# broadinstitute/permutect

Measured on AMD Instinct MI355X. Metric: read-sets/sec (train fwd+bwd), higher is better.
Workload: dtype f32 (fp32 accumulate; fwd: 2 x f16 pieces per operand = 23 bits; bwd: 2 x bf16 pieces = 16 bits)

## Files before the change

include/permutect_amd.h:

```cpp
#ifndef PERMUTECT_AMD_H
#define PERMUTECT_AMD_H

#include <stddef.h>
#include <stdint.h>

#ifdef __cplusplus
extern "C" {
#endif

#define PMT_ABI_VERSION 12

#define PMT_FAULT_JOIN 1
#define PMT_FAULT_F16_RANGE 2
#define PMT_FAULT_PLAN 4

#define PMT_OK 0
#define PMT_E_INVALID (-1)
#define PMT_E_UNSUPPORTED (-2)
#define PMT_E_CAPACITY (-3)
#define PMT_E_LAUNCH (-4)
#define PMT_E_WORKSPACE (-5)

#ifndef PMT_MAX_WIDTH
#define PMT_MAX_WIDTH 64
#endif
#ifndef PMT_MAX_HALF_FFN
#define PMT_MAX_HALF_FFN 16
#endif
#define PMT_MAX_CLUSTERS 16
#define PMT_MAX_OPS 8
#define PMT_MAX_ROW_INPUT 128
#define PMT_MAX_CNN_TAPS 192
#define PMT_ROWS_INFO 0
#define PMT_ROWS_ALT_COUNT 1
#define PMT_ROWS_SOURCE 2
#define PMT_MAX_SKIP_LAYERS 4
#define PMT_MAX_BLOCKS 16
#define PMT_MAX_LINEAR 96
#ifndef PMT_GROUP_WAVES
#define PMT_GROUP_WAVES 8
#endif
#define PMT_GROUP_TILES (2 * PMT_GROUP_WAVES)
#define PMT_GROUP_MAX_SETS (8 * PMT_GROUP_WAVES)
#define PMT_TILE 16

#define PMT_READS_PACKED_U8 0
#define PMT_READS_F16 1
#define PMT_READS_F32 2

typedef struct PmtLinear {
    int32_t in_dim, out_dim;
    int32_t w_frag;
    int32_t wt_frag;
    int32_t b_pvec;
    int32_t w_src;
    int32_t b_src;
    int32_t out_split;
    int32_t wb_frag;
    int32_t wtb_frag;
    int32_t wh_frag;
    int32_t emit_tab;
} PmtLinear;

#define PMT_OP_LINEAR 0
#define PMT_OP_SKIP 1
typedef struct PmtOp {
    int32_t kind;
    int32_t n_layers;
    int32_t selu_after;
    int32_t alpha_src;
    int32_t lin[PMT_MAX_SKIP_LAYERS];
} PmtOp;

typedef struct PmtMlp {
    int32_t n_ops, in_dim, out_dim;
    int32_t dropout;
    PmtOp ops[PMT_MAX_OPS];
} PmtMlp;

typedef struct PmtBlock {
    int32_t norm_w_pvec, norm_b_pvec;
    int32_t norm_w_src, norm_b_src;
    int32_t proj1[2], proj2[2];
    int32_t sgu_norm_w_pvec, sgu_norm_b_pvec;
    int32_t sgu_norm_w_src, sgu_norm_b_src;
    int32_t alpha_src[2], beta_src[2];
    int32_t gamma_src;
    int32_t ref_reg_pvec, ref_reg_src;
    int32_t reg_weight_phi;
} PmtBlock;

typedef struct PmtHead {
    int32_t stdev_e_phi;
    int32_t dirs_ke_phi;
    int32_t art_stdev_k_phi;
    int32_t log_w_k_phi;
    int32_t mu_k_src;
    int32_t sigma_k_phi;
    int32_t lambda_k_phi;
    int32_t reserved;
} PmtHead;

#define PMT_MAX_CNN_LAYERS 12
#define PMT_CNN_CONV 0
#define PMT_CNN_POOL 1
#define PMT_CNN_LEAKY_RELU 2
#define PMT_CNN_SELU 3
#define PMT_CNN_FLATTEN 4
#define PMT_CNN_LINEAR 5
typedef struct PmtCnnLayer {
    int32_t kind;
    int32_t in_ch, in_len, out_ch, out_len;
    int32_t kernel, stride, padding, dilation;
    int32_t w_src, b_src;
    int32_t in_off, out_off;
    int32_t lin;
    int32_t reserved[2];
} PmtCnnLayer;
typedef struct PmtCnn {
    int32_t n_layers;
    int32_t seq_len;
    int32_t out_dim;
    int32_t max_act;
    int32_t sum_act;
    int32_t reserved[3];
    PmtCnnLayer layers[PMT_MAX_CNN_LAYERS];
} PmtCnn;

typedef struct PmtModel {
    int32_t abi_version;
    int32_t num_read_features;
    int32_t read_embed_dim;
    int32_t variant_embed_dim;
    int32_t d_model;
    int32_t d_ffn;
    int32_t num_blocks;
    int32_t feature_dim;
    int32_t num_clusters;
    int32_t n_linear;
    int32_t theta_size, phi_size, packed_size;
    int32_t translation_src;
    int32_t translation_pvec;
    int32_t rotation_lin;
    PmtMlp read_mlp;
    PmtMlp reducer;
    PmtMlp row_mlp[3];
    PmtBlock blocks[PMT_MAX_BLOCKS];
    PmtHead head;
    PmtCnn cnn;
    PmtLinear lin[PMT_MAX_LINEAR];
    int32_t force_shape;
    int32_t force_cnn;
    int32_t cnn_debug;
    int32_t emit_base;
    int32_t emit_len;
    float dropout_p;
} PmtModel;

typedef struct PmtBatch {
    int32_t num_variants;
    int32_t num_groups;
    int32_t read_format;
    int32_t read_row_bytes;
    const void* reads;
    const int64_t* read_index;
    const int32_t* ref_offsets;
    const int32_t* alt_offsets;
    const float* variant_embed;
    const int32_t* group_start;
    const int32_t* group_tile_base;
    int64_t total_tiles;
    int32_t* debug_flags;
    const int32_t* group_span;
    const int32_t* num_groups_dev;
    const int32_t* set_groups;
    uint64_t dropout_seed;
    int32_t* join_fault;
} PmtBatch;

typedef struct PmtOutputs {
    float* logits_b;
    float* logits_bk;
    float* features_be;
    float* ref_features_be;
} PmtOutputs;

typedef struct PmtOutputGrads {
    const float* d_logits_b;
    const float* d_logits_bk;
    const float* d_features_be;
    const float* d_ref_features_be;
} PmtOutputGrads;

typedef struct PmtAdamW {
    float lr, beta1, beta2, eps, weight_decay, max_grad_norm;
    int32_t step;
    int32_t reserved;
} PmtAdamW;
#define PMT_STEP_ON_DEVICE (-1)
#define PMT_STEP_SLOT 1000


int pmt_abi_version(void);

int pmt_shape_info(int32_t* nine);
int pmt_shape_id(const struct PmtModel* m);
int pmt_limits(int32_t* four);

int pmt_build_id(char* out, int32_t capacity);

int pmt_struct_bytes(int which);

int pmt_model_check(const PmtModel* model);

#define PMT_PHI_EXP 0
#define PMT_PHI_BOUNDED 1
#define PMT_PHI_UNIT_ROWS 2
#define PMT_PHI_LOG_SOFTMAX 3
#define PMT_PHI_ORTHOGONAL 4
#define PMT_MAX_PHI_SEGS 48
#define PMT_MAX_ORTHO_DIM 32
typedef struct PmtPhiSeg {
    int32_t kind, theta_off, phi_off, rows, cols, reserved;
    float p0, p1;
    int32_t base_rs, base_cs;
    const float* base;
} PmtPhiSeg;
typedef struct PmtPhiProgram {
    int32_t n_segs, reserved;
    PmtPhiSeg seg[PMT_MAX_PHI_SEGS];
} PmtPhiProgram;

int pmt_phi_forward(const PmtPhiProgram* prog, const float* theta, float* phi, void* stream);
int pmt_phi_backward(const PmtPhiProgram* prog, const float* theta, const float* phi, const float* grad_phi,
                     float* grad_theta, void* stream);

typedef struct PmtIntColumn {
    const void* ptr;
    int64_t stride;
    int32_t elem_bytes, reserved;
} PmtIntColumn;

typedef struct PmtBinning {
    int32_t num_sources, num_variant_types, num_ref_bins, num_alt_bins, count_bin_skip, max_ref_count, max_alt_count, reserved;
} PmtBinning;

typedef struct PmtDownsample {
    int32_t num_variants;
    int32_t reference_alt_gather;
    uint64_t seed;
    int64_t force_random;
    const int32_t* ref_offsets;
    const int32_t* alt_offsets;
    const float* ref_weights_b4;
    const float* alt_weights_b4;
    const float* ref_fracs_in;
    const float* alt_fracs_in;
    const float* ref_weight_table;
    const float* alt_weight_table;
    PmtIntColumn labels, variant_types, sources;
    PmtBinning bins;
} PmtDownsample;
int pmt_downsample_counts(const PmtDownsample* args, float* ref_fracs, float* alt_fracs, int32_t* new_ref_counts,
                          int32_t* new_alt_counts, void* stream);
int pmt_downsample_index(const PmtDownsample* args, const float* ref_fracs, const float* alt_fracs,
                         const int32_t* new_ref_offsets, const int32_t* new_alt_offsets, int64_t* read_index, void* stream);

#define PMT_FIT_MAX_STEPS 200000
int pmt_downsample_fit(const float* counts_slvra, int32_t num_sources, const float* ref_trans_kry, const float* alt_trans_haz,
                       float* ref_logits_slvrak, float* alt_logits_slvrah, int32_t steps, double lr, double beta1, double beta2,
                       double eps, double weight_decay, float* loss_before_after, void* stream);

int pmt_spectra_fit(const int32_t* variant_types, const int32_t* depths, const int32_t* alt_counts, int32_t n, float* log_alpha_dv,
                    float* log_beta_dv, int32_t batch_size, int32_t epochs, double lr, double beta1, double beta2, double eps,
                    void* stream);

#define PMT_POSTERIOR_RAW 80
#define PMT_POSTERIOR_PARTIAL 128
typedef struct PmtPosteriorRows {
    int64_t n;
    const int32_t *variant_types, *depths, *alt_counts, *normal_depths, *normal_alt_counts, *contexts;
    const float *seq_error_log_lks, *normal_seq_error_log_lks, *allele_frequencies, *mafs, *normal_mafs, *artifact_logits;
} PmtPosteriorRows;
typedef struct PmtPosteriorParams {
    const float *log_priors_vc, *snv_log_priors_rrra, *raw;
    int32_t use_context, no_germline, has_het_beta;
    float het_beta;
} PmtPosteriorParams;
int pmt_posterior_forward(const PmtPosteriorRows* rows, int64_t first, int64_t count, const PmtPosteriorParams* params, float* log_priors_bc,
                          float* spectra_log_lks_bc, float* normal_log_lks_bc, float* log_posteriors_bc, void* stream);
int pmt_posterior_step(const PmtPosteriorRows* rows, int64_t first, int64_t count, const PmtPosteriorParams* params, float* partials,
                       int32_t num_partial_rows, void* stream);
int pmt_posterior_update(const float* partials, int32_t num_partial_rows, int64_t count, float* raw, float* adam_m, float* adam_v, int64_t step,
                         double lr, double beta1, double beta2, double eps, float* totals_tc, double* loss_sum, void* stream);

typedef struct PmtLossArgs {
    int32_t num_variants, num_clusters, num_sources, reserved;
    float max_outlier_logit;
    float max_alt_count;
    const float* logits_b;
    const float* logits_bk;
    const float* alt_count_raw;
    const float* source_logits;
    const int64_t* labels;
    int64_t label_stride;
    const int64_t* alt_counts;
    int64_t alt_count_stride;
    const int64_t* sources;
    int64_t source_stride;
    const float* weights;
    const float* source_weights;
} PmtLossArgs;
typedef struct PmtLossOutputs {
    float* supervised_b;
    float* unsupervised_b;
    float* alt_count_b;
    float* source_b;
    float* total_b;
} PmtLossOutputs;
typedef struct PmtLossInputGrads {
    float* d_logits_b;
    float* d_logits_bk;
    float* d_alt_count_raw;
    float* d_source_logits;
} PmtLossInputGrads;
int pmt_losses_forward(const PmtLossArgs* args, const PmtLossOutputs* out, void* stream);
int pmt_losses_backward(const PmtLossArgs* args, const PmtLossOutputs* grad_out, const PmtLossInputGrads* grad_in, void* stream);

typedef struct PmtRecordArgs {
    int32_t num_variants, num_bins;
    int32_t num_variant_types, num_ref_bins, num_alt_bins, count_bin_skip, max_ref_count, max_alt_count;
    PmtIntColumn labels, variant_types, sources, ref_counts, alt_counts;
    const float* weights;
    const float* source_weights;
    const float* supervised_b;
    const float* unsupervised_b;
    const float* alt_count_b;
    const float* source_b;
} PmtRecordArgs;
int pmt_record_losses(const PmtRecordArgs* args, float* histograms, void* stream);

typedef struct PmtEvalArgs {
    int32_t num_variants, epoch_index;
    int32_t num_logit_bins, min_logit, max_logit, logit_bin_skip;
    PmtBinning bins;
    PmtIntColumn labels, variant_types, sources, ref_counts, alt_counts;
    const float* logits_b;
    const float* weights_b;
    int64_t nhist;
} PmtEvalArgs;
int pmt_record_evaluation(const PmtEvalArgs* args, float* flat, void* stream);

typedef struct PmtBalanceArgs {
    int32_t num_variants, recompute;
    float attenuation;
    int32_t reserved;
    PmtBinning bins;
    PmtIntColumn labels, variant_types, sources, ref_counts, alt_counts;
    const float* logits_b;
    float* counts;
    float* pseudo_counts;
    const float* weights_in;
    const float* unlabeled_weights_in;
    const float* source_weights_in;
    float* weights_out;
    float* unlabeled_weights_out;
    float* source_weights_out;
    float* weights_b;
    float* source_weights_b;
} PmtBalanceArgs;
int pmt_balance_step(const PmtBalanceArgs* args, void* stream);

int pmt_posterior_rows(const float* float_rows, int64_t float_stride, int32_t n_scalars, int32_t logit_col, const float* logits_b,
                       const float* features_be, int32_t e, const int64_t* dest_ids, int32_t n, float* block, int64_t block_stride,
                       void* stream);

int pmt_plan_groups(const int32_t* ref_counts, const int32_t* alt_counts, int32_t num_variants,
                    int32_t* group_start, int32_t* group_tile_base, int32_t* bad_variant);

int pmt_plan_groups_device(const int32_t* ref_offsets, const int32_t* alt_offsets, int32_t num_variants, int32_t* group_start,
                           int32_t* group_tile_base, int32_t capacity, int32_t* num_groups_dev, int32_t* fault, int32_t* scratch,
                           void* stream);
int pmt_plan_device_chunks(int32_t num_variants);

int pmt_pack_order(const int32_t* ref_counts, const int32_t* alt_counts, int32_t num_variants, int32_t window, int32_t* order);
int pmt_pack_order_batches(const int32_t* ref_counts, const int32_t* alt_counts, int32_t num_variants, int32_t batch,
                           int32_t window, int32_t threads, int32_t* order);

int pmt_plan_groups_split(const int32_t* ref_counts, const int32_t* alt_counts, int32_t num_variants, int32_t* span,
                          int32_t* tile_base, int32_t max_groups, int32_t* needs_layered);

size_t pmt_layered_scratch_floats(const PmtModel* model, int64_t total_tiles, int32_t num_variants);

int pmt_forward_layered(const PmtModel* model_host, const PmtModel* model_dev, const float* theta, const float* phi,
                        const float* packed, const PmtBatch* batch, const PmtOutputs* out, float* stash, float* scratch,
                        void* stream);

size_t pmt_layered_backward_scratch_floats(const PmtModel* model, int64_t total_tiles, int32_t num_variants);

int pmt_backward_layered(const PmtModel* model_host, const PmtModel* model_dev, const float* theta, const float* phi,
                         const float* packed, const PmtBatch* batch, const PmtOutputs* out, const PmtOutputGrads* dout,
                         const float* stash, float* scratch, float* grad_theta, float* grad_phi, float* grad_variant_embed,
                         float* grad_partials, int32_t num_partials, void* stream);

size_t pmt_stash_bytes(const PmtModel* model, int64_t total_tiles, int32_t num_variants);


int pmt_pack_params(const PmtModel* model_host, const PmtModel* model_dev, const float* theta, const float* phi,
                    float* packed, void* stream);

int pmt_scan_counts(const void* ref_counts, const void* alt_counts, int32_t count_elem_bytes, int64_t count_stride,
                    int32_t num_variants, int32_t* ref_offsets, int32_t* alt_offsets, void* stream);

int pmt_build_read_index(const int64_t* row_start, const int32_t* ref_offsets, const int32_t* alt_offsets,
                         int32_t num_variants, int64_t* read_index, void* stream);

int pmt_compose_batch(const int16_t* chunk_ints, int32_t int_cols, const void* chunk_floats_f16, int32_t float_cols,
                      const int64_t* chunk_row_start, const int64_t* ids, int32_t num_variants, int32_t ref_col, int32_t alt_col,
                      int64_t* int_tensor, float* float_tensor, int64_t* row_start, int32_t* ref_offsets, int32_t* alt_offsets,
                      int64_t* read_index, void* stream);
int pmt_compose_batch_planned(const int16_t* chunk_ints, int32_t int_cols, const void* chunk_floats_f16, int32_t float_cols,
                              const int64_t* chunk_row_start, const int64_t* ids, int32_t num_variants,
                              const int32_t* ref_offsets, const int32_t* alt_offsets, int64_t* int_tensor, float* float_tensor,
                              int64_t* row_start, int64_t* read_index, void* stream);

int pmt_host_copy(void* dst, const void* src, size_t bytes, int32_t threads);
int pmt_host_copy_rows(void* dst, const void* src, int64_t rows, int64_t row_bytes, int64_t zero_offset, int64_t zero_bytes,
                       int32_t threads);
int pmt_prepare_chunk(const int16_t* ints, int64_t row_stride, int32_t ref_col, int32_t alt_col, int32_t n, int32_t shuffle,
                      uint64_t seed, int32_t batch, int32_t window, int32_t threads, int32_t* ref_host, int32_t* alt_host,
                      int64_t* ids, int32_t* plans, int64_t plans_capacity, int32_t* batch_info, int32_t* offsets);

int pmt_forward(const PmtModel* model_host, const PmtModel* model_dev, const float* theta, const float* phi,
                const float* packed, const PmtBatch* batch, const PmtOutputs* out, float* stash, void* stream);

int pmt_backward(const PmtModel* model_host, const PmtModel* model_dev, const float* theta, const float* phi,
                 const float* packed, const PmtBatch* batch, const PmtOutputs* out, const PmtOutputGrads* dout,
                 const float* stash, float* grad_theta, float* grad_phi, float* grad_variant_embed, float* grad_partials,
                 int32_t num_partials, void* stream);

int pmt_dropout_mask(uint64_t seed, float p, int32_t lin, int64_t row0, int64_t rows, int32_t width, float* out);

size_t pmt_rows_stash_bytes(const PmtModel* model, int which, int32_t n_rows);
int pmt_rows_forward(const PmtModel* model_host, const PmtModel* model_dev, int which, const float* theta,
                     const float* packed, const float* in, int64_t in_stride, int32_t n_rows, float* out,
                     int64_t out_stride, float* stash, uint64_t dropout_seed, void* stream);
int pmt_rows_backward(const PmtModel* model_host, const PmtModel* model_dev, int which, const float* theta,
                      const float* packed, const float* in, int64_t in_stride, int32_t n_rows, const float* d_out,
                      int64_t d_out_stride, const float* stash, float* grad_theta, float* d_in, int64_t d_in_stride,
                      float d_in_scale, float* workspace, size_t workspace_floats, uint64_t dropout_seed, void* stream);
size_t pmt_rows_workspace_floats(const PmtModel* model_host, int which);

int pmt_cnn_forward(const PmtModel* model_host, const PmtModel* model_dev, const float* theta, const float* packed,
                    const int64_t* haplotypes, int64_t hap_stride, int32_t n, float* out, int64_t out_stride, float* stash,
                    void* stream);
size_t pmt_cnn_stash_floats(const PmtModel* model_host);
int pmt_cnn_backward(const PmtModel* model_host, const PmtModel* model_dev, const float* theta, const float* packed,
                     const int64_t* haplotypes, int64_t hap_stride, int32_t n, const float* d_out, int64_t d_out_stride,
                     const float* stash, float* grad_theta, float* workspace, size_t workspace_floats, void* stream);
size_t pmt_cnn_workspace_floats(const PmtModel* model_host);

int pmt_clip_adamw(float* theta, const float* grad, float* exp_avg, float* exp_avg_sq, int64_t n,
                   const PmtAdamW* hyper, float* scratch, float* grad_norm_out, void* stream);

#ifdef __cplusplus
}
#endif
#endif
```

permutect_amd/architecture/artifact_model.py:

```python
from __future__ import annotations

from typing import Optional

import torch
from torch import Tensor, nn

from permutect_amd import constants
from permutect_amd.architecture import modules as M
from permutect_amd.data.batch import Batch
from permutect_amd.data.datum import Data
from permutect_amd.engine import lib as L
from permutect_amd.engine.runtime import (HaplotypeCnnFunction, LossesFunction, PhiFunction, ReadSetEngine, ReadSetFunction,
                                          RowsMlpFunction, VariantEmbedFunction)
from permutect_amd.enums import Epoch
from permutect_amd.parameters import ModelParameters, install_pickle_alias

_BCE = nn.BCEWithLogitsLoss(reduction="none")


def gpu_if_available() -> torch.device:
    return torch.device("cuda" if torch.cuda.is_available() else "cpu")


class BatchOutput:

    def __init__(self, features_be: Tensor, ref_features_be: Tensor, logits_b: Tensor, logits_bk: Tensor,
                 weights: Tensor, source_weights: Tensor):
        self.features_be = features_be
        self.ref_features_be = ref_features_be
        self.logits_b = logits_b
        self.logits_bk = logits_bk
        self.weights = weights
        self.source_weights = source_weights

    @property
    def artifact_probs_b(self) -> Tensor:
        return torch.sigmoid(self.logits_b)

    @property
    def outlier_binary_logits(self) -> Tensor:
        lk = self.logits_bk
        nonoutlier = torch.logsumexp(torch.cat((lk[:, 0:1], lk[:, 2:]), dim=-1), dim=-1)
        return lk[:, 1] - nonoutlier


class BatchLosses:

    def __init__(self, supervised_losses_b, unsupervised_losses_b, alt_count_losses_b, source_prediction_losses_b,
                 total_losses_b):
        self.supervised_losses_b = supervised_losses_b
        self.unsupervised_losses_b = unsupervised_losses_b
        self.alt_count_losses_b = alt_count_losses_b
        self.source_prediction_losses_b = source_prediction_losses_b
        self.total_losses_b = total_losses_b
        self.total_loss = torch.sum(total_losses_b)


class SetMeansView:

    def __init__(self, means_be: Tensor, lengths_b: Tensor):
        self._means, self.lengths_b = means_be, lengths_b

    def means_over_sets(self) -> Tensor:
        return self._means

    def batch_size(self) -> int:
        return len(self.lengths_b)


class ArtifactModel(nn.Module):
    def __init__(self, params: ModelParameters, num_read_features: int, num_info_features: int,
                 haplotypes_length: int, device=None):
        super().__init__()
        if device is None:
            device = gpu_if_available()
        self._device = torch.device(device)
        if self._device.type == "cuda" and self._device.index is None:
            self._device = torch.device("cuda", torch.cuda.current_device())
        self._dtype = torch.float32
        self._haplotypes_length = haplotypes_length
        self._params = params

        self.read_embedding = M.MLP([num_read_features] + params.read_layers, params.batch_normalize, params.dropout_p)
        self.info_embedding = M.MLP([num_info_features] + params.info_layers, params.batch_normalize, params.dropout_p)
        self.haplotypes_cnn = M.DNASequenceConvolution(params.ref_seq_layer_strings, haplotypes_length // 2)
        embedding_dim = (self.read_embedding.output_dimension() + self.info_embedding.output_dimension()
                         + self.haplotypes_cnn.output_dimension())
        self.ref_alt_reads_encoder = M.GatedRefAltMLP(embedding_dim, params.self_attention_hidden_dimension,
                                                      params.num_self_attention_layers)
        self.reducer = M.MLP([embedding_dim] + params.aggregation_layers, params.batch_normalize, params.dropout_p)
        e = self.reducer.output_dimension()
        self.pre_clustering_transform = M.EuclideanTransformation(e)
        self.feature_clustering = M.FeatureClustering(e, params.num_artifact_clusters)
        self.alt_count_predictor = M.Adversarial(M.MLP([e] + [30, -1, -1, -1, 1]), adversarial_strength=0.01)
        self.alt_count_loss_func = nn.MSELoss(reduction="none")
        self.source_predictor = M.Adversarial(M.MLP([e] + [1], params.batch_normalize, params.dropout_p), 0.01)
        self.num_sources = 1

        self.to(device=self._device, dtype=self._dtype)
        self._engine: Optional[ReadSetEngine] = None

    def engine(self) -> ReadSetEngine:
        if self._engine is None:
            with torch.inference_mode(False):
                self._engine = ReadSetEngine(self, self._device)
        return self._engine

    def _invalidate_engine(self):
        self._engine = None

    def reset_source_predictor(self, num_sources: int = 1):
        hidden = [] if num_sources == 1 else [-1, -1]
        layers = [self.reducer.output_dimension()] + hidden + [num_sources]
        self.source_predictor = M.Adversarial(
            M.MLP(layers, self._params.batch_normalize, self._params.dropout_p), 0.01
        ).to(device=self._device, dtype=self._dtype)
        self.num_sources = num_sources
        self._invalidate_engine()

    def ref_alt_seq_embedding_dimension(self) -> int:
        return self.haplotypes_cnn.output_dimension()

    def haplotypes_length(self) -> int:
        return self._haplotypes_length

    def calibration_parameters(self):
        fc = self.feature_clustering
        return [fc.parametrizations.nonartifact_stdev_e.original, fc.parametrizations.artifact_stdev_k.original]

    def set_epoch_type(self, epoch_type: Epoch):
        train = epoch_type == Epoch.TRAIN
        self.train(train)
        for p in self.parameters():
            p.requires_grad_(train)

    def forward(self, batch: Batch):
        pass

    def variant_embedding(self, batch: Batch) -> Tensor:
        eng = self.engine()
        return VariantEmbedFunction.apply(eng, batch.get_info_be(), batch.get_haplotypes_bs(), eng.trigger)

    def _cnn_has_batchnorm(self) -> bool:
        flag = self.__dict__.get("_cnn_bn_flag")
        if flag is None:
            flag = self.__dict__["_cnn_bn_flag"] = any(isinstance(m, nn.BatchNorm1d) for m in self.haplotypes_cnn.modules())
        return flag

    def _encode(self, batch: Batch):
        if self.training and self._cnn_has_batchnorm():
            raise NotImplementedError("permutect_amd runs a haplotype CNN with batch_norm tokens in eval mode only (model.eval() under "
                                      "no_grad / inference_mode: filter_variants, evaluation); training with BatchNorm statistics is not built")
        if self.training and self._params.batch_normalize:
            raise NotImplementedError("permutect_amd runs a batch_normalize model in eval mode only (model.eval(): filter_variants, "
                                      "evaluation); training with BatchNorm statistics is not built")
        eng = self.engine()
        eng.draw_dropout_seed(self.training)
        if batch.size() == 0:
            d, dev = eng.plan.desc, self._device
            z = lambda *shape: torch.zeros(*shape, dtype=torch.float32, device=dev)
            return (z(0), z(0, d.num_clusters + 2), z(0, d.feature_dim), z(0, d.feature_dim)), z(0, d.variant_embed_dim)
        key = None if torch.is_grad_enabled() else eng.params_key()
        if key is not None and eng.packed_for is not None and eng.packed_for[0] == key:
            phi = eng.packed_for[1]
        else:
            prog = eng.plan.phi_program(self)
            phi = eng.plan.materialize_phi(self) if prog is None else PhiFunction.apply(eng, prog, eng.trigger)
            eng.pack(phi.detach().contiguous())
            eng.packed_for = (key, phi.detach()) if (key is not None and not torch.is_grad_enabled()) else None
        variant_embed = self.variant_embedding(batch)
        outs = ReadSetFunction.apply(eng, batch, phi, variant_embed)
        return outs, variant_embed

    def calculate_features(self, batch: Batch, weight_range: float = 0):
        (logits_b, logits_bk, feats, ref_feats), ve = self._encode(batch)
        e_hap = self.haplotypes_cnn.output_dimension()
        return (SetMeansView(ref_feats, batch.get(Data.REF_COUNT)), SetMeansView(feats, batch.get(Data.ALT_COUNT)),
                ve[:, ve.shape[1] - e_hap:])

    def compute_batch_output(self, batch: Batch, balancer=None) -> BatchOutput:
        (logits_b, logits_bk, feats, ref_feats), _ = self._encode(batch)
        if balancer is None:
            weights_b = source_weights = torch.ones_like(logits_b)
        elif logits_b.is_cuda and hasattr(balancer, "weights_from_logits"):
            weights_b, source_weights = balancer.weights_from_logits(batch, logits_b)
        else:
            weights_b, source_weights_b = balancer.process_batch_and_compute_weights(
                batch, artifact_probs_b=torch.sigmoid(logits_b).detach())
            source_weights = weights_b * source_weights_b
        return BatchOutput(features_be=feats, ref_features_be=ref_feats, logits_b=logits_b, logits_bk=logits_bk,
                           weights=weights_b, source_weights=source_weights)

    def compute_source_prediction_losses(self, features_be: Tensor, batch: Batch) -> Tensor:
        if self.num_sources > 1:
            eng = self.engine()
            logits = RowsMlpFunction.apply(eng, L.ROWS_SOURCE, features_be, eng.trigger,
                                           float(self.source_predictor.gradient_reversal.alpha))
            probs = torch.softmax(logits, dim=-1)
            targets = torch.nn.functional.one_hot(batch.get(Data.SOURCE).long(), self.num_sources)
            return torch.sum(torch.square(probs - targets), dim=-1)
        return torch.zeros(batch.size(), device=self._device, dtype=self._dtype)

    def compute_alt_count_losses(self, features_be: Tensor, batch: Batch) -> Tensor:
        eng = self.engine()
        raw = RowsMlpFunction.apply(eng, L.ROWS_ALT_COUNT, features_be, eng.trigger,
                                    float(self.alt_count_predictor.gradient_reversal.alpha))
        pred = torch.sigmoid(raw.view(-1))
        target = batch.get(Data.ALT_COUNT).to(dtype=pred.dtype) / constants.MAX_ALT_COUNT
        return self.alt_count_loss_func(pred, target)

    def compute_batch_losses(self, output: BatchOutput, batch: Batch) -> BatchLosses:
        eng = self.engine()
        alt_raw = RowsMlpFunction.apply(eng, L.ROWS_ALT_COUNT, output.features_be, eng.trigger,
                                        float(self.alt_count_predictor.gradient_reversal.alpha))
        source_logits, sources = None, None
        if self.num_sources > 1:
            source_logits = RowsMlpFunction.apply(eng, L.ROWS_SOURCE, output.features_be, eng.trigger,
                                                  float(self.source_predictor.gradient_reversal.alpha))
            sources = batch.get(Data.SOURCE).long()
        sup, unsup, alt, src, total = LossesFunction.apply(
            eng, output.logits_b, output.logits_bk, alt_raw, source_logits, batch.get(Data.LABEL).long(),
            batch.get(Data.ALT_COUNT).long(), sources, output.weights, output.source_weights)
        return BatchLosses(sup, unsup, alt, src, total)

    def compute_batch_losses_torch(self, output: BatchOutput, batch: Batch) -> BatchLosses:
        labels_b = batch.get_training_labels()
        is_labeled_b = batch.get_is_labeled_mask()
        supervised = is_labeled_b * _BCE(output.logits_b, labels_b)
        clipped = torch.clip(output.outlier_binary_logits, max=constants.MAX_OUTLIER_LOGIT)
        unsupervised = (1 - is_labeled_b) * _BCE(clipped, torch.zeros_like(clipped))
        alt_count = self.compute_alt_count_losses(output.features_be, batch)
        source = self.compute_source_prediction_losses(output.features_be, batch)
        total = output.weights * (supervised + unsupervised + alt_count) + output.source_weights * source
        return BatchLosses(supervised, unsupervised, alt_count, source, total)

    def make_dict_for_saving(self, artifact_log_priors=None, artifact_spectra=None):
        state = {k: v.detach().clone() for k, v in self.state_dict().items()}
        return {
            constants.STATE_DICT_NAME: state,
            constants.HYPERPARAMS_NAME: self._params,
            constants.NUM_READ_FEATURES_NAME: self.read_embedding.input_dimension(),
            constants.NUM_INFO_FEATURES_NAME: self.info_embedding.input_dimension(),
            constants.REF_SEQUENCE_LENGTH_NAME: self.haplotypes_length(),
            constants.ARTIFACT_LOG_PRIORS_NAME: artifact_log_priors,
            constants.ARTIFACT_SPECTRA_STATE_DICT_NAME: None if artifact_spectra is None else artifact_spectra.state_dict(),
        }

    def save_model(self, path, artifact_log_priors=None, artifact_spectra=None):
        self.reset_source_predictor()
        install_pickle_alias()
        torch.save(self.make_dict_for_saving(artifact_log_priors, artifact_spectra), path)


def load_model(path, device: torch.device = None):
    if device is None:
        device = gpu_if_available()
    install_pickle_alias()
    with torch.serialization.safe_globals([ModelParameters]):
        saved = torch.load(path, map_location=device, weights_only=True)
    model = ArtifactModel(saved[constants.HYPERPARAMS_NAME], num_read_features=saved[constants.NUM_READ_FEATURES_NAME],
                          num_info_features=saved[constants.NUM_INFO_FEATURES_NAME],
                          haplotypes_length=saved[constants.REF_SEQUENCE_LENGTH_NAME], device=device)
    model.load_state_dict(saved[constants.STATE_DICT_NAME])
    model.to(model._dtype)
    return model, saved[constants.ARTIFACT_LOG_PRIORS_NAME], saved[constants.ARTIFACT_SPECTRA_STATE_DICT_NAME]
```

permutect_amd/csrc/pmt_losses.hip:

```cpp
#include <hip/hip_runtime.h>
#include <math.h>

#include "permutect_amd.h"

#define LOSS_THREADS 256

__device__ __forceinline__ float softplus_f(float x) { return fmaxf(x, 0.f) + log1pf(expf(-fabsf(x))); }
__device__ __forceinline__ float sigmoid_f(float x) { return 1.0f / (1.0f + expf(-x)); }

struct OutlierLogit {
    float o;
    float mx, se;
};
__device__ __forceinline__ OutlierLogit outlier_logit(const float* __restrict__ lk, int K) {
    OutlierLogit r;
    r.mx = lk[0];
    for (int k = 0; k < K; ++k) r.mx = fmaxf(r.mx, lk[2 + k]);
    r.se = expf(lk[0] - r.mx);
    for (int k = 0; k < K; ++k) r.se += expf(lk[2 + k] - r.mx);
    r.o = lk[1] - (r.mx + logf(r.se));
    return r;
}

__global__ __launch_bounds__(LOSS_THREADS) void pmt_losses_forward_kernel(PmtLossArgs a, PmtLossOutputs out) {
    const int b = blockIdx.x * LOSS_THREADS + threadIdx.x;
    if (b >= a.num_variants) return;
    const int K = a.num_clusters, S = a.num_sources;
    const long long label = a.labels[(size_t)b * a.label_stride];
    const float is_labeled = label != 2 ? 1.f : 0.f;
    const float target = label == 0 ? 1.f : (label == 2 ? 0.5f : 0.f);
    const float x = a.logits_b[b];
    const float sup = is_labeled * (fmaxf(x, 0.f) - x * target + log1pf(expf(-fabsf(x))));
    const OutlierLogit ol = outlier_logit(a.logits_bk + (size_t)b * (K + 2), K);
    const float unsup = (1.f - is_labeled) * softplus_f(fminf(ol.o, a.max_outlier_logit));
    const float pred = sigmoid_f(a.alt_count_raw[b]);
    const float tgt = (float)a.alt_counts[(size_t)b * a.alt_count_stride] / a.max_alt_count;
    const float altl = (pred - tgt) * (pred - tgt);
    float src = 0.f;
    if (S > 1 && a.source_logits != nullptr) {
        const float* sl = a.source_logits + (size_t)b * S;
        const long long sid = a.sources[(size_t)b * a.source_stride];
        float mx = sl[0];
        for (int s = 1; s < S; ++s) mx = fmaxf(mx, sl[s]);
        float se = 0.f;
        for (int s = 0; s < S; ++s) se += expf(sl[s] - mx);
        for (int s = 0; s < S; ++s) {
            const float d = expf(sl[s] - mx) / se - (s == sid ? 1.f : 0.f);
            src += d * d;
        }
    }
    out.supervised_b[b] = sup;
    out.unsupervised_b[b] = unsup;
    out.alt_count_b[b] = altl;
    out.source_b[b] = src;
    out.total_b[b] = a.weights[b] * (sup + unsup + altl) + a.source_weights[b] * src;
}

__global__ __launch_bounds__(LOSS_THREADS) void pmt_losses_backward_kernel(PmtLossArgs a, PmtLossOutputs g, PmtLossInputGrads d) {
    const int b = blockIdx.x * LOSS_THREADS + threadIdx.x;
    if (b >= a.num_variants) return;
    const int K = a.num_clusters, S = a.num_sources;
    const float gt = g.total_b ? g.total_b[b] : 0.f;
    const float g_sup = (g.supervised_b ? g.supervised_b[b] : 0.f) + gt * a.weights[b];
    const float g_unsup = (g.unsupervised_b ? g.unsupervised_b[b] : 0.f) + gt * a.weights[b];
    const float g_alt = (g.alt_count_b ? g.alt_count_b[b] : 0.f) + gt * a.weights[b];
    const float g_src = (g.source_b ? g.source_b[b] : 0.f) + gt * a.source_weights[b];
    const long long label = a.labels[(size_t)b * a.label_stride];
    const float is_labeled = label != 2 ? 1.f : 0.f;
    const float target = label == 0 ? 1.f : (label == 2 ? 0.5f : 0.f);
    d.d_logits_b[b] = g_sup * is_labeled * (sigmoid_f(a.logits_b[b]) - target);
    const float* lk = a.logits_bk + (size_t)b * (K + 2);
    float* dlk = d.d_logits_bk + (size_t)b * (K + 2);
    const OutlierLogit ol = outlier_logit(lk, K);
    const float go = ol.o <= a.max_outlier_logit ? g_unsup * (1.f - is_labeled) * sigmoid_f(ol.o) : 0.f;
    dlk[1] = go;
    dlk[0] = -go * expf(lk[0] - ol.mx) / ol.se;
    for (int k = 0; k < K; ++k) dlk[2 + k] = -go * expf(lk[2 + k] - ol.mx) / ol.se;
    const float pred = sigmoid_f(a.alt_count_raw[b]);
    const float tgt = (float)a.alt_counts[(size_t)b * a.alt_count_stride] / a.max_alt_count;
    d.d_alt_count_raw[b] = g_alt * 2.f * (pred - tgt) * pred * (1.f - pred);
    if (S > 1 && a.source_logits != nullptr && d.d_source_logits != nullptr) {
        const float* sl = a.source_logits + (size_t)b * S;
        float* dsl = d.d_source_logits + (size_t)b * S;
        const long long sid = a.sources[(size_t)b * a.source_stride];
        float mx = sl[0];
        for (int s = 1; s < S; ++s) mx = fmaxf(mx, sl[s]);
        float se = 0.f;
        for (int s = 0; s < S; ++s) se += expf(sl[s] - mx);
        float dot = 0.f;
        for (int s = 0; s < S; ++s) {
            const float p = expf(sl[s] - mx) / se;
            dot += 2.f * (p - (s == sid ? 1.f : 0.f)) * p;
        }
        for (int s = 0; s < S; ++s) {
            const float p = expf(sl[s] - mx) / se;
            dsl[s] = g_src * (2.f * (p - (s == sid ? 1.f : 0.f)) * p - p * dot);
        }
    }
}

static int loss_args_check(const PmtLossArgs* a) {
    if (!a || a->num_variants < 0 || a->num_clusters < 0 || a->num_clusters > PMT_MAX_CLUSTERS || a->num_sources < 1) return PMT_E_INVALID;
    if (a->num_variants == 0) return PMT_OK;
    if (!a->logits_b || !a->logits_bk || !a->alt_count_raw || !a->labels || !a->alt_counts || !a->weights || !a->source_weights)
        return PMT_E_INVALID;
    if (a->num_sources > 1 && a->source_logits && !a->sources) return PMT_E_INVALID;
    return PMT_OK;
}

extern "C" int pmt_losses_forward(const PmtLossArgs* args, const PmtLossOutputs* out, void* stream) {
    const int rc = loss_args_check(args);
    if (rc) return rc;
    if (!out || !out->supervised_b || !out->unsupervised_b || !out->alt_count_b || !out->source_b || !out->total_b) return PMT_E_INVALID;
    if (args->num_variants == 0) return PMT_OK;
    hipLaunchKernelGGL(pmt_losses_forward_kernel, dim3((args->num_variants + LOSS_THREADS - 1) / LOSS_THREADS), dim3(LOSS_THREADS), 0,
                       reinterpret_cast<hipStream_t>(stream), *args, *out);
    return hipGetLastError() == hipSuccess ? PMT_OK : PMT_E_LAUNCH;
}

extern "C" int pmt_losses_backward(const PmtLossArgs* args, const PmtLossOutputs* grad_out, const PmtLossInputGrads* grad_in,
                                   void* stream) {
    const int rc = loss_args_check(args);
    if (rc) return rc;
    if (!grad_out || !grad_in || !grad_in->d_logits_b || !grad_in->d_logits_bk || !grad_in->d_alt_count_raw) return PMT_E_INVALID;
    if (args->num_variants == 0) return PMT_OK;
    hipLaunchKernelGGL(pmt_losses_backward_kernel, dim3((args->num_variants + LOSS_THREADS - 1) / LOSS_THREADS), dim3(LOSS_THREADS), 0,
                       reinterpret_cast<hipStream_t>(stream), *args, *grad_out, *grad_in);
    return hipGetLastError() == hipSuccess ? PMT_OK : PMT_E_LAUNCH;
}

#define REC_THREADS 256
#define REC_MAX_BINS 2048

__device__ __forceinline__ long long rec_col_at(const PmtIntColumn& c, int i) {
    if (c.ptr == nullptr) return 0;
    return c.elem_bytes == 8 ? reinterpret_cast<const long long*>(c.ptr)[(size_t)i * c.stride]
                             : (long long)reinterpret_cast<const int*>(c.ptr)[(size_t)i * c.stride];
}

__global__ __launch_bounds__(REC_THREADS) void pmt_record_losses_kernel(PmtRecordArgs a, float* __restrict__ hist) {
    __shared__ float sh[6][REC_MAX_BINS];
    const int nb = a.num_bins;
    for (int i = threadIdx.x; i < 6 * REC_MAX_BINS; i += REC_THREADS) (&sh[0][0])[i] = 0.f;
    __syncthreads();
    const int b = blockIdx.x * REC_THREADS + threadIdx.x;
    if (b < a.num_variants) {
        const long long label = rec_col_at(a.labels, b), vt = rec_col_at(a.variant_types, b), src = rec_col_at(a.sources, b);
        const long long nr = rec_col_at(a.ref_counts, b), na = rec_col_at(a.alt_counts, b);
        const int rbin = (int)min(nr, (long long)a.max_ref_count) / a.count_bin_skip;
        const int abin = ((int)min(na, (long long)a.max_alt_count) - 1) / a.count_bin_skip;
        const int idx = (int)((((src * 3 + label) * a.num_variant_types + vt) * a.num_ref_bins + rbin) * a.num_alt_bins + abin);
        if (idx >= 0 && idx < nb) {
            const float is_labeled = label != 2 ? 1.f : 0.f;
            const float w = a.weights[b], sw = a.source_weights[b];
            const float lw = is_labeled * w, uw = (1.f - is_labeled) * w;
            atomicAdd(&sh[0][idx], a.supervised_b[b] * lw + a.unsupervised_b[b] * uw);
            atomicAdd(&sh[1][idx], lw + uw);
            atomicAdd(&sh[2][idx], a.alt_count_b[b] * w);
            atomicAdd(&sh[3][idx], w);
            atomicAdd(&sh[4][idx], a.source_b[b] * sw);
            atomicAdd(&sh[5][idx], sw);
        }
    }
    __syncthreads();
    for (int i = threadIdx.x; i < 6 * nb; i += REC_THREADS) {
        const int hsel = i / nb, j = i - hsel * nb;
        const float v = sh[hsel][j];
        if (v != 0.f) atomicAdd(&hist[(size_t)hsel * nb + j], v);
    }
}

extern "C" int pmt_record_losses(const PmtRecordArgs* args, float* histograms, void* stream) {
    if (!args || !histograms || args->num_variants < 0 || args->num_bins < 1 || args->num_bins > REC_MAX_BINS) return PMT_E_INVALID;
    if (args->num_variants == 0) return PMT_OK;
    for (const PmtIntColumn* c : {&args->labels, &args->variant_types, &args->sources, &args->ref_counts, &args->alt_counts})
        if (c->ptr != nullptr && c->elem_bytes != 4 && c->elem_bytes != 8) return PMT_E_INVALID;
    if (!args->labels.ptr || !args->variant_types.ptr || !args->ref_counts.ptr || !args->alt_counts.ptr || !args->weights || !args->source_weights ||
        !args->supervised_b || !args->unsupervised_b || !args->alt_count_b || !args->source_b || args->count_bin_skip < 1)
        return PMT_E_INVALID;
    hipLaunchKernelGGL(pmt_record_losses_kernel, dim3((args->num_variants + REC_THREADS - 1) / REC_THREADS), dim3(REC_THREADS), 0,
                       reinterpret_cast<hipStream_t>(stream), *args, histograms);
    return hipGetLastError() == hipSuccess ? PMT_OK : PMT_E_LAUNCH;
}

__global__ __launch_bounds__(256) void pmt_posterior_rows_kernel(const float* __restrict__ float_rows, long long float_stride, int n_scalars,
                                                                 int logit_col, const float* __restrict__ logits_b,
                                                                 const float* __restrict__ features_be, int e,
                                                                 const long long* __restrict__ dest_ids, int n, float* __restrict__ block,
                                                                 long long block_stride) {
    const int width = n_scalars + e;
    for (long long i = (long long)blockIdx.x * 256 + threadIdx.x; i < (long long)n * width; i += (long long)gridDim.x * 256) {
        const int v = (int)(i / width), c = (int)(i - (long long)v * width);
        const long long row = dest_ids ? dest_ids[v] : v;
        float x;
        if (c < n_scalars) {
            const float raw = c == logit_col ? logits_b[v] : float_rows[(long long)v * float_stride + c];
            x = (float)(_Float16)raw;
        } else {
            x = features_be[(long long)v * e + (c - n_scalars)];
        }
        block[row * block_stride + c] = x;
    }
}

extern "C" int pmt_posterior_rows(const float* float_rows, int64_t float_stride, int32_t n_scalars, int32_t logit_col, const float* logits_b,
                                  const float* features_be, int32_t e, const int64_t* dest_ids, int32_t n, float* block, int64_t block_stride,
                                  void* stream) {
    if (!float_rows || !logits_b || !features_be || !block || n < 0 || n_scalars < 1 || e < 0 || logit_col < 0 || logit_col >= n_scalars ||
        block_stride < n_scalars + e)
        return PMT_E_INVALID;
    if (n == 0) return PMT_OK;
    const long long work = (long long)n * (n_scalars + e);
    const int grid = (int)((work + 255) / 256 < 4096 ? (work + 255) / 256 : 4096);
    hipLaunchKernelGGL(pmt_posterior_rows_kernel, dim3(grid), dim3(256), 0, reinterpret_cast<hipStream_t>(stream), float_rows, (long long)float_stride,
                       n_scalars, logit_col, logits_b, features_be, e, reinterpret_cast<const long long*>(dest_ids), n, block, (long long)block_stride);
    return hipGetLastError() == hipSuccess ? PMT_OK : PMT_E_LAUNCH;
}
```

permutect_amd/csrc/pmt_phi.hip:

```cpp
#include <hip/hip_runtime.h>
#include <math.h>

#include "permutect_amd.h"

#define PHI_THREADS 256
#define PHI_MAXN (2 * PMT_MAX_ORTHO_DIM)

__device__ double block_max(double v, double* red) {
    const int tid = threadIdx.x;
    red[tid] = v;
    __syncthreads();
    for (int s = PHI_THREADS / 2; s > 0; s >>= 1) {
        if (tid < s) red[tid] = fmax(red[tid], red[tid + s]);
        __syncthreads();
    }
    const double r = red[0];
    __syncthreads();
    return r;
}
__device__ double block_sum(double v, double* red) {
    const int tid = threadIdx.x;
    red[tid] = v;
    __syncthreads();
    for (int s = PHI_THREADS / 2; s > 0; s >>= 1) {
        if (tid < s) red[tid] += red[tid + s];
        __syncthreads();
    }
    const double r = red[0];
    __syncthreads();
    return r;
}

__device__ void matmul(double* __restrict__ Cm, const double* __restrict__ A, const double* __restrict__ B, int N, double scale) {
    for (int idx = threadIdx.x; idx < N * N; idx += PHI_THREADS) {
        const int i = idx / N, j = idx - i * N;
        double a0 = 0.0, a1 = 0.0, a2 = 0.0, a3 = 0.0;
        const double* ar = A + i * N;
        const double* bc = B + j;
        int k = 0;
        for (; k + 3 < N; k += 4) {
            a0 += ar[k] * bc[k * N];
            a1 += ar[k + 1] * bc[(k + 1) * N];
            a2 += ar[k + 2] * bc[(k + 2) * N];
            a3 += ar[k + 3] * bc[(k + 3) * N];
        }
        for (; k < N; ++k) a0 += ar[k] * bc[k * N];
        Cm[idx] = ((a0 + a1) + (a2 + a3)) * scale;
    }
    __syncthreads();
}

__device__ void expm_inplace(double* S, double* B, double* P, double* T, int N, double* red) {
    double colsum = 0.0;
    if (threadIdx.x < N)
        for (int i = 0; i < N; ++i) colsum += fabs(S[i * N + threadIdx.x]);
    const double norm1 = block_max(colsum, red);
    int s = 0;
    if (norm1 > 0.5) s = (int)ceil(log2(norm1 / 0.5));
    const double scale = ldexp(1.0, -s);
    for (int idx = threadIdx.x; idx < N * N; idx += PHI_THREADS) {
        const double b = S[idx] * scale;
        B[idx] = b;
        P[idx] = b;
        const int i = idx / N, j = idx - i * N;
        S[idx] = b + (i == j ? 1.0 : 0.0);
    }
    __syncthreads();
    for (int k = 2; k <= 12; ++k) {
        matmul(T, P, B, N, 1.0 / (double)k);
        for (int idx = threadIdx.x; idx < N * N; idx += PHI_THREADS) {
            P[idx] = T[idx];
            S[idx] += T[idx];
        }
        __syncthreads();
    }
    for (int q = 0; q < s; ++q) {
        matmul(T, S, S, N, 1.0);
        for (int idx = threadIdx.x; idx < N * N; idx += PHI_THREADS) S[idx] = T[idx];
        __syncthreads();
    }
}

struct PhiShared {
    double m[4][PHI_MAXN * PHI_MAXN];
    double red[PHI_THREADS];
};
static_assert(sizeof(PhiShared) <= 160 * 1024, "LDS budget");

__global__ __launch_bounds__(PHI_THREADS) void pmt_phi_forward_kernel(PmtPhiProgram prog, const float* __restrict__ theta,
                                                                       float* __restrict__ phi) {
    __shared__ __attribute__((aligned(16))) PhiShared sh;
    const PmtPhiSeg sg = prog.seg[blockIdx.x];
    const float* x = theta + sg.theta_off;
    float* y = phi + sg.phi_off;
    const int tid = threadIdx.x, n = sg.rows * sg.cols;
    if (sg.kind == PMT_PHI_EXP) {
        for (int i = tid; i < n; i += PHI_THREADS) y[i] = expf(x[i]);
    } else if (sg.kind == PMT_PHI_BOUNDED) {
        for (int i = tid; i < n; i += PHI_THREADS) y[i] = sg.p1 * (1.0f / (1.0f + expf(-x[i]))) + sg.p0;
    } else if (sg.kind == PMT_PHI_UNIT_ROWS) {
        for (int r = 0; r < sg.rows; ++r) {
            double q = 0.0;
            for (int i = tid; i < sg.cols; i += PHI_THREADS) q += (double)x[r * sg.cols + i] * (double)x[r * sg.cols + i];
            const float norm = (float)sqrt(block_sum(q, sh.red));
            for (int i = tid; i < sg.cols; i += PHI_THREADS) y[r * sg.cols + i] = x[r * sg.cols + i] / norm;
        }
    } else if (sg.kind == PMT_PHI_LOG_SOFTMAX) {
        for (int r = 0; r < sg.rows; ++r) {
            double mx = -INFINITY;
            for (int i = tid; i < sg.cols; i += PHI_THREADS) mx = fmax(mx, (double)x[r * sg.cols + i]);
            mx = block_max(mx, sh.red);
            double se = 0.0;
            for (int i = tid; i < sg.cols; i += PHI_THREADS) se += exp((double)x[r * sg.cols + i] - mx);
            const double lse = mx + log(block_sum(se, sh.red));
            for (int i = tid; i < sg.cols; i += PHI_THREADS) y[r * sg.cols + i] = (float)((double)x[r * sg.cols + i] - lse);
        }
    } else if (sg.kind == PMT_PHI_ORTHOGONAL) {
        const int N = sg.rows;
        double* S = sh.m[0];
        for (int idx = tid; idx < N * N; idx += PHI_THREADS) {
            const int i = idx / N, j = idx - i * N;
            S[idx] = i > j ? (double)x[i * N + j] : (i < j ? -(double)x[j * N + i] : 0.0);
        }
        __syncthreads();
        expm_inplace(S, sh.m[1], sh.m[2], sh.m[3], N, sh.red);
        for (int idx = tid; idx < N * N; idx += PHI_THREADS) {
            const int i = idx / N, j = idx - i * N;
            double acc = 0.0;
            if (sg.base != nullptr) {
                for (int k = 0; k < N; ++k) acc += (double)sg.base[i * sg.base_rs + k * sg.base_cs] * S[k * N + j];
            } else {
                acc = S[idx];
            }
            y[idx] = (float)acc;
        }
    }
}

__global__ __launch_bounds__(PHI_THREADS) void pmt_phi_backward_kernel(PmtPhiProgram prog, const float* __restrict__ theta,
                                                                        const float* __restrict__ phi,
                                                                        const float* __restrict__ gphi,
                                                                        float* __restrict__ gtheta) {
    __shared__ __attribute__((aligned(16))) PhiShared sh;
    const PmtPhiSeg sg = prog.seg[blockIdx.x];
    const float* x = theta + sg.theta_off;
    const float* y = phi + sg.phi_off;
    const float* gy = gphi + sg.phi_off;
    float* gx = gtheta + sg.theta_off;
    const int tid = threadIdx.x, n = sg.rows * sg.cols;
    if (sg.kind == PMT_PHI_EXP) {
        for (int i = tid; i < n; i += PHI_THREADS) gx[i] += gy[i] * y[i];
    } else if (sg.kind == PMT_PHI_BOUNDED) {
        for (int i = tid; i < n; i += PHI_THREADS) {
            const float s = 1.0f / (1.0f + expf(-x[i]));
            gx[i] += gy[i] * sg.p1 * s * (1.0f - s);
        }
    } else if (sg.kind == PMT_PHI_UNIT_ROWS) {
        for (int r = 0; r < sg.rows; ++r) {
            double q = 0.0, d = 0.0;
            for (int i = tid; i < sg.cols; i += PHI_THREADS) {
                q += (double)x[r * sg.cols + i] * (double)x[r * sg.cols + i];
                d += (double)y[r * sg.cols + i] * (double)gy[r * sg.cols + i];
            }
            const double norm = sqrt(block_sum(q, sh.red));
            const double dot = block_sum(d, sh.red);
            for (int i = tid; i < sg.cols; i += PHI_THREADS)
                gx[r * sg.cols + i] += (float)(((double)gy[r * sg.cols + i] - (double)y[r * sg.cols + i] * dot) / norm);
        }
    } else if (sg.kind == PMT_PHI_LOG_SOFTMAX) {
        for (int r = 0; r < sg.rows; ++r) {
            double g = 0.0;
            for (int i = tid; i < sg.cols; i += PHI_THREADS) g += (double)gy[r * sg.cols + i];
            const double gsum = block_sum(g, sh.red);
            for (int i = tid; i < sg.cols; i += PHI_THREADS)
                gx[r * sg.cols + i] += (float)((double)gy[r * sg.cols + i] - exp((double)y[r * sg.cols + i]) * gsum);
        }
    } else if (sg.kind == PMT_PHI_ORTHOGONAL) {
        const int nn = sg.rows, N = 2 * nn;
        double* S = sh.m[0];
        double* G = sh.m[1];
        for (int idx = tid; idx < nn * nn; idx += PHI_THREADS) {
            const int i = idx / nn, j = idx - i * nn;
            double acc = 0.0;
            if (sg.base != nullptr) {
                for (int k = 0; k < nn; ++k) acc += (double)sg.base[k * sg.base_rs + i * sg.base_cs] * (double)gy[k * nn + j];
            } else {
                acc = (double)gy[idx];
            }
            G[idx] = acc;
        }
        __syncthreads();
        for (int idx = tid; idx < N * N; idx += PHI_THREADS) {
            const int i = idx / N, j = idx - i * N;
            const int bi = i % nn, bj = j % nn;
            double v = 0.0;
            if ((i < nn) == (j < nn)) {
                v = bi > bj ? -(double)x[bi * nn + bj] : (bi < bj ? (double)x[bj * nn + bi] : 0.0);
            } else if (i < nn) {
                v = G[bi * nn + bj];
            }
            S[idx] = v;
        }
        __syncthreads();
        double* B = sh.m[1];
        expm_inplace(S, B, sh.m[2], sh.m[3], N, sh.red);
        for (int idx = tid; idx < nn * nn; idx += PHI_THREADS) {
            const int i = idx / nn, j = idx - i * nn;
            if (i > j) gx[idx] += (float)(S[i * N + nn + j] - S[j * N + nn + i]);
        }
    }
}

static int phi_check(const PmtPhiProgram* p) {
    if (!p || p->n_segs < 0 || p->n_segs > PMT_MAX_PHI_SEGS) return PMT_E_INVALID;
    for (int i = 0; i < p->n_segs; ++i) {
        const PmtPhiSeg* s = &p->seg[i];
        if (s->kind < PMT_PHI_EXP || s->kind > PMT_PHI_ORTHOGONAL || s->rows < 1 || s->cols < 1 || s->theta_off < 0 || s->phi_off < 0)
            return PMT_E_INVALID;
        if (s->kind == PMT_PHI_ORTHOGONAL && (s->rows != s->cols || s->rows > PMT_MAX_ORTHO_DIM)) return PMT_E_UNSUPPORTED;
    }
    return PMT_OK;
}

extern "C" int pmt_phi_forward(const PmtPhiProgram* prog, const float* theta, float* phi, void* stream) {
    const int rc = phi_check(prog);
    if (rc) return rc;
    if (!theta || !phi) return PMT_E_INVALID;
    if (prog->n_segs == 0) return PMT_OK;
    hipLaunchKernelGGL(pmt_phi_forward_kernel, dim3(prog->n_segs), dim3(PHI_THREADS), 0, reinterpret_cast<hipStream_t>(stream),
                       *prog, theta, phi);
    return hipGetLastError() == hipSuccess ? PMT_OK : PMT_E_LAUNCH;
}

extern "C" int pmt_phi_backward(const PmtPhiProgram* prog, const float* theta, const float* phi, const float* grad_phi,
                                float* grad_theta, void* stream) {
    const int rc = phi_check(prog);
    if (rc) return rc;
    if (!theta || !phi || !grad_phi || !grad_theta) return PMT_E_INVALID;
    if (prog->n_segs == 0) return PMT_OK;
    hipLaunchKernelGGL(pmt_phi_backward_kernel, dim3(prog->n_segs), dim3(PHI_THREADS), 0, reinterpret_cast<hipStream_t>(stream),
                       *prog, theta, phi, grad_phi, grad_theta);
    return hipGetLastError() == hipSuccess ? PMT_OK : PMT_E_LAUNCH;
}
```

permutect_amd/engine/lib.py:

```python
from __future__ import annotations

import ctypes as C
import os

_HERE = os.path.dirname(os.path.dirname(os.path.abspath(__file__)))
LIB_PATH = os.environ.get("PMT_LIB", os.path.join(_HERE, "libpermutect_amd.so"))

ABI_VERSION = 12
MAX_WIDTH, MAX_HALF_FFN, MAX_CLUSTERS = 64, 16, 16
MAX_HALF_FFN_WIDE = 32
MAX_WIDTH_WIDE = 128
MAX_ROW_INPUT = 128
MAX_CNN_TAPS = 192
ROWS_INFO, ROWS_ALT_COUNT, ROWS_SOURCE = 0, 1, 2
MAX_OPS, MAX_SKIP_LAYERS, MAX_BLOCKS, MAX_LINEAR = 8, 4, 16, 96
GROUP_WAVES = int(os.environ.get("PMT_GROUP_WAVES", 8))
GROUP_TILES, GROUP_MAX_SETS, TILE = 2 * GROUP_WAVES, 8 * GROUP_WAVES, 16
READS_PACKED_U8, READS_F16, READS_F32 = 0, 1, 2
OP_LINEAR, OP_SKIP = 0, 1
SLOT_FLOATS = 4 * 256

POSTERIOR_RAW, POSTERIOR_PARTIAL = 80, 128

STEP_ON_DEVICE, STEP_SLOT = -1, 1000
E_INVALID, E_UNSUPPORTED, E_CAPACITY, E_LAUNCH, E_WORKSPACE = -1, -2, -3, -4, -5
_ERR = {-1: "invalid argument/descriptor", -2: "configuration not supported by the gfx950 kernels",
        -3: "a read set exceeds the register-resident group capacity", -4: "HIP launch failure",
        -5: "workspace too small"}

i32, i64, vp = C.c_int32, C.c_int64, C.c_void_p


class PmtLinear(C.Structure):
    _fields_ = [("in_dim", i32), ("out_dim", i32), ("w_frag", i32), ("wt_frag", i32), ("b_pvec", i32),
                ("w_src", i32), ("b_src", i32), ("out_split", i32), ("wb_frag", i32), ("wtb_frag", i32), ("wh_frag", i32), ("emit_tab", i32)]


class PmtOp(C.Structure):
    _fields_ = [("kind", i32), ("n_layers", i32), ("selu_after", i32), ("alpha_src", i32),
                ("lin", i32 * MAX_SKIP_LAYERS)]


class PmtMlp(C.Structure):
    _fields_ = [("n_ops", i32), ("in_dim", i32), ("out_dim", i32), ("dropout", i32), ("ops", PmtOp * MAX_OPS)]


class PmtBlock(C.Structure):
    _fields_ = [("norm_w_pvec", i32), ("norm_b_pvec", i32), ("norm_w_src", i32), ("norm_b_src", i32),
                ("proj1", i32 * 2), ("proj2", i32 * 2),
                ("sgu_norm_w_pvec", i32), ("sgu_norm_b_pvec", i32), ("sgu_norm_w_src", i32), ("sgu_norm_b_src", i32),
                ("alpha_src", i32 * 2), ("beta_src", i32 * 2), ("gamma_src", i32),
                ("ref_reg_pvec", i32), ("ref_reg_src", i32), ("reg_weight_phi", i32)]


class PmtHead(C.Structure):
    _fields_ = [("stdev_e_phi", i32), ("dirs_ke_phi", i32), ("art_stdev_k_phi", i32), ("log_w_k_phi", i32),
                ("mu_k_src", i32), ("sigma_k_phi", i32), ("lambda_k_phi", i32), ("reserved", i32)]


MAX_CNN_LAYERS = 12
CNN_CONV, CNN_POOL, CNN_LEAKY_RELU, CNN_SELU, CNN_FLATTEN, CNN_LINEAR = range(6)


class PmtCnnLayer(C.Structure):
    _fields_ = [("kind", i32), ("in_ch", i32), ("in_len", i32), ("out_ch", i32), ("out_len", i32),
                ("kernel", i32), ("stride", i32), ("padding", i32), ("dilation", i32), ("w_src", i32), ("b_src", i32),
                ("in_off", i32), ("out_off", i32), ("lin", i32), ("reserved", i32 * 2)]


class PmtCnn(C.Structure):
    _fields_ = [("n_layers", i32), ("seq_len", i32), ("out_dim", i32), ("max_act", i32), ("sum_act", i32),
                ("reserved", i32 * 3), ("layers", PmtCnnLayer * MAX_CNN_LAYERS)]


class PmtModel(C.Structure):
    _fields_ = [("abi_version", i32), ("num_read_features", i32), ("read_embed_dim", i32),
                ("variant_embed_dim", i32), ("d_model", i32), ("d_ffn", i32), ("num_blocks", i32),
                ("feature_dim", i32), ("num_clusters", i32), ("n_linear", i32),
                ("theta_size", i32), ("phi_size", i32), ("packed_size", i32),
                ("translation_src", i32), ("translation_pvec", i32), ("rotation_lin", i32),
                ("read_mlp", PmtMlp), ("reducer", PmtMlp), ("row_mlp", PmtMlp * 3), ("blocks", PmtBlock * MAX_BLOCKS), ("head", PmtHead), ("cnn", PmtCnn),
                ("lin", PmtLinear * MAX_LINEAR),
                ("force_shape", i32), ("force_cnn", i32), ("cnn_debug", i32), ("emit_base", i32), ("emit_len", i32),
                ("dropout_p", C.c_float)]


class PmtBatch(C.Structure):
    _fields_ = [("num_variants", i32), ("num_groups", i32), ("read_format", i32), ("read_row_bytes", i32),
                ("reads", vp), ("read_index", vp), ("ref_offsets", vp), ("alt_offsets", vp), ("variant_embed", vp),
                ("group_start", vp), ("group_tile_base", vp), ("total_tiles", i64), ("debug_flags", vp), ("group_span", vp),
                ("num_groups_dev", vp), ("set_groups", vp), ("dropout_seed", C.c_uint64), ("join_fault", vp)]


class PmtOutputs(C.Structure):
    _fields_ = [("logits_b", vp), ("logits_bk", vp), ("features_be", vp), ("ref_features_be", vp)]


class PmtOutputGrads(C.Structure):
    _fields_ = [("d_logits_b", vp), ("d_logits_bk", vp), ("d_features_be", vp), ("d_ref_features_be", vp)]


class PmtAdamW(C.Structure):
    _fields_ = [("lr", C.c_float), ("beta1", C.c_float), ("beta2", C.c_float), ("eps", C.c_float),
                ("weight_decay", C.c_float), ("max_grad_norm", C.c_float), ("step", i32), ("reserved", i32)]


PHI_EXP, PHI_BOUNDED, PHI_UNIT_ROWS, PHI_LOG_SOFTMAX, PHI_ORTHOGONAL = range(5)
MAX_PHI_SEGS, MAX_ORTHO_DIM = 48, 32


class PmtPhiSeg(C.Structure):
    _fields_ = [("kind", i32), ("theta_off", i32), ("phi_off", i32), ("rows", i32), ("cols", i32), ("reserved", i32),
                ("p0", C.c_float), ("p1", C.c_float), ("base_rs", i32), ("base_cs", i32), ("base", vp)]


class PmtPhiProgram(C.Structure):
    _fields_ = [("n_segs", i32), ("reserved", i32), ("seg", PmtPhiSeg * MAX_PHI_SEGS)]


class PmtIntColumn(C.Structure):
    _fields_ = [("ptr", vp), ("stride", i64), ("elem_bytes", i32), ("reserved", i32)]


class PmtBinning(C.Structure):
    _fields_ = [("num_sources", i32), ("num_variant_types", i32), ("num_ref_bins", i32), ("num_alt_bins", i32),
                ("count_bin_skip", i32), ("max_ref_count", i32), ("max_alt_count", i32), ("reserved", i32)]


def int_column(t) -> PmtIntColumn:
    c = PmtIntColumn()
    if t is None:
        return c
    assert t.dim() == 1 and t.element_size() in (4, 8) and not t.is_floating_point(), (t.shape, t.dtype)
    c.ptr, c.stride, c.elem_bytes = t.data_ptr(), (t.stride(0) if t.numel() > 1 else 1), t.element_size()
    return c


class PmtDownsample(C.Structure):
    _fields_ = [("num_variants", i32), ("reference_alt_gather", i32), ("seed", C.c_uint64), ("force_random", i64),
                ("ref_offsets", vp), ("alt_offsets", vp), ("ref_weights_b4", vp), ("alt_weights_b4", vp),
                ("ref_fracs_in", vp), ("alt_fracs_in", vp), ("ref_weight_table", vp), ("alt_weight_table", vp),
                ("labels", PmtIntColumn), ("variant_types", PmtIntColumn), ("sources", PmtIntColumn), ("bins", PmtBinning)]


class PmtBalanceArgs(C.Structure):
    _fields_ = [("num_variants", i32), ("recompute", i32), ("attenuation", C.c_float), ("reserved", i32), ("bins", PmtBinning),
                ("labels", PmtIntColumn), ("variant_types", PmtIntColumn), ("sources", PmtIntColumn), ("ref_counts", PmtIntColumn),
                ("alt_counts", PmtIntColumn), ("logits_b", vp), ("counts", vp), ("pseudo_counts", vp),
                ("weights_in", vp), ("unlabeled_weights_in", vp), ("source_weights_in", vp),
                ("weights_out", vp), ("unlabeled_weights_out", vp), ("source_weights_out", vp),
                ("weights_b", vp), ("source_weights_b", vp)]


class PmtEvalArgs(C.Structure):
    _fields_ = [("num_variants", i32), ("epoch_index", i32), ("num_logit_bins", i32), ("min_logit", i32), ("max_logit", i32),
                ("logit_bin_skip", i32), ("bins", PmtBinning), ("labels", PmtIntColumn), ("variant_types", PmtIntColumn),
                ("sources", PmtIntColumn), ("ref_counts", PmtIntColumn), ("alt_counts", PmtIntColumn), ("logits_b", vp), ("weights_b", vp),
                ("nhist", i64)]


class PmtRecordArgs(C.Structure):
    _fields_ = [("num_variants", i32), ("num_bins", i32), ("num_variant_types", i32), ("num_ref_bins", i32),
                ("num_alt_bins", i32), ("count_bin_skip", i32), ("max_ref_count", i32), ("max_alt_count", i32),
                ("labels", PmtIntColumn), ("variant_types", PmtIntColumn), ("sources", PmtIntColumn), ("ref_counts", PmtIntColumn),
                ("alt_counts", PmtIntColumn), ("weights", vp), ("source_weights", vp),
                ("supervised_b", vp), ("unsupervised_b", vp), ("alt_count_b", vp), ("source_b", vp)]


class PmtLossArgs(C.Structure):
    _fields_ = [("num_variants", i32), ("num_clusters", i32), ("num_sources", i32), ("reserved", i32),
                ("max_outlier_logit", C.c_float), ("max_alt_count", C.c_float),
                ("logits_b", vp), ("logits_bk", vp), ("alt_count_raw", vp), ("source_logits", vp),
                ("labels", vp), ("label_stride", i64), ("alt_counts", vp), ("alt_count_stride", i64),
                ("sources", vp), ("source_stride", i64), ("weights", vp), ("source_weights", vp)]


class PmtLossOutputs(C.Structure):
    _fields_ = [("supervised_b", vp), ("unsupervised_b", vp), ("alt_count_b", vp), ("source_b", vp), ("total_b", vp)]


class PmtLossInputGrads(C.Structure):
    _fields_ = [("d_logits_b", vp), ("d_logits_bk", vp), ("d_alt_count_raw", vp), ("d_source_logits", vp)]


class PmtPosteriorRows(C.Structure):
    _fields_ = [("n", i64), ("variant_types", vp), ("depths", vp), ("alt_counts", vp), ("normal_depths", vp), ("normal_alt_counts", vp),
                ("contexts", vp), ("seq_error_log_lks", vp), ("normal_seq_error_log_lks", vp), ("allele_frequencies", vp), ("mafs", vp),
                ("normal_mafs", vp), ("artifact_logits", vp)]


class PmtPosteriorParams(C.Structure):
    _fields_ = [("log_priors_vc", vp), ("snv_log_priors_rrra", vp), ("raw", vp), ("use_context", i32), ("no_germline", i32),
                ("has_het_beta", i32), ("het_beta", C.c_float)]


EXPORTS = ["pmt_abi_version", "pmt_build_id", "pmt_shape_info", "pmt_shape_id", "pmt_limits", "pmt_struct_bytes", "pmt_model_check", "pmt_plan_groups", "pmt_plan_groups_device", "pmt_plan_device_chunks", "pmt_stash_bytes", "pmt_pack_params",
           "pmt_scan_counts", "pmt_forward", "pmt_backward", "pmt_clip_adamw",
           "pmt_dropout_mask", "pmt_rows_stash_bytes", "pmt_rows_forward", "pmt_rows_backward", "pmt_rows_workspace_floats", "pmt_cnn_forward", "pmt_cnn_backward", "pmt_cnn_stash_floats", "pmt_cnn_workspace_floats",
           "pmt_phi_forward", "pmt_phi_backward", "pmt_build_read_index", "pmt_losses_forward", "pmt_losses_backward",
           "pmt_downsample_counts", "pmt_downsample_index", "pmt_downsample_fit", "pmt_spectra_fit", "pmt_posterior_forward", "pmt_posterior_step", "pmt_posterior_update", "pmt_record_losses", "pmt_record_evaluation", "pmt_balance_step", "pmt_posterior_rows",
           "pmt_plan_groups_split", "pmt_layered_scratch_floats", "pmt_forward_layered",
           "pmt_layered_backward_scratch_floats", "pmt_backward_layered", "pmt_host_copy", "pmt_pack_order", "pmt_pack_order_batches", "pmt_prepare_chunk", "pmt_host_copy_rows", "pmt_compose_batch", "pmt_compose_batch_planned"]

_lib = None
_libs = {}


class PmtError(RuntimeError):
    pass


def check(rc: int, what: str) -> int:
    if rc < 0:
        raise PmtError(f"{what} failed: {_ERR.get(rc, rc)} (code {rc})")
    return rc


def load(path: str = None) -> C.CDLL:
    global _lib
    if path is None and _lib is not None:
        return _lib
    path = LIB_PATH if path is None else path
    if path in _libs:
        return _libs[path]
    if not os.path.exists(path):
        raise PmtError(f"{path} not found: build it with `python -c 'import __graft_entry__ as g; g.build()'` "
                       f"or `make -C permutect_amd/csrc`.  permutect_amd has no CPU fallback.")
    lib = C.CDLL(path)
    P = C.POINTER
    lib.pmt_abi_version.restype = i32
    lib.pmt_model_check.argtypes = [P(PmtModel)]
    lib.pmt_plan_groups.argtypes = [vp, vp, i32, vp, vp, P(i32)]
    lib.pmt_plan_groups_device.argtypes = [vp, vp, i32, vp, vp, i32, vp, vp, vp, vp]
    lib.pmt_plan_device_chunks.argtypes = [i32]
    lib.pmt_stash_bytes.argtypes = [P(PmtModel), i64, i32]
    lib.pmt_stash_bytes.restype = C.c_size_t
    lib.pmt_pack_params.argtypes = [P(PmtModel), vp, vp, vp, vp, vp]
    lib.pmt_scan_counts.argtypes = [vp, vp, i32, i64, i32, vp, vp, vp]
    lib.pmt_forward.argtypes = [P(PmtModel), vp, vp, vp, vp, P(PmtBatch), P(PmtOutputs), vp, vp]
    lib.pmt_backward.argtypes = [P(PmtModel), vp, vp, vp, vp, P(PmtBatch), P(PmtOutputs), P(PmtOutputGrads), vp, vp, vp, vp, vp, i32, vp]
    lib.pmt_clip_adamw.argtypes = [vp, vp, vp, vp, i64, P(PmtAdamW), vp, vp, vp]
    lib.pmt_cnn_forward.argtypes = [P(PmtModel), vp, vp, vp, vp, i64, i32, vp, i64, vp, vp]
    lib.pmt_cnn_backward.argtypes = [P(PmtModel), vp, vp, vp, vp, i64, i32, vp, i64, vp, vp, vp, C.c_size_t, vp]
    lib.pmt_cnn_workspace_floats.argtypes = [P(PmtModel)]
    lib.pmt_cnn_workspace_floats.restype = C.c_size_t
    lib.pmt_cnn_stash_floats.argtypes = [P(PmtModel)]
    lib.pmt_cnn_stash_floats.restype = C.c_size_t
    lib.pmt_rows_stash_bytes.argtypes = [P(PmtModel), i32, i32]
    lib.pmt_rows_stash_bytes.restype = C.c_size_t
    lib.pmt_rows_forward.argtypes = [P(PmtModel), vp, i32, vp, vp, vp, i64, i32, vp, i64, vp, C.c_uint64, vp]
    lib.pmt_rows_backward.argtypes = [P(PmtModel), vp, i32, vp, vp, vp, i64, i32, vp, i64, vp, vp, vp, i64, C.c_float, vp, C.c_size_t, C.c_uint64, vp]
    lib.pmt_dropout_mask.argtypes = [C.c_uint64, C.c_float, i32, i64, i64, i32, vp]
    lib.pmt_rows_workspace_floats.argtypes = [P(PmtModel), i32]
    lib.pmt_rows_workspace_floats.restype = C.c_size_t
    lib.pmt_build_read_index.argtypes = [vp, vp, vp, i32, vp, vp]
    lib.pmt_record_losses.argtypes = [P(PmtRecordArgs), vp, vp]
    lib.pmt_plan_groups_split.argtypes = [vp, vp, i32, vp, vp, i32, P(i32)]
    lib.pmt_layered_scratch_floats.argtypes = [P(PmtModel), i64, i32]
    lib.pmt_layered_scratch_floats.restype = C.c_size_t
    lib.pmt_forward_layered.argtypes = [P(PmtModel), vp, vp, vp, vp, P(PmtBatch), P(PmtOutputs), vp, vp, vp]
    lib.pmt_host_copy.argtypes = [vp, vp, C.c_size_t, i32]
    lib.pmt_host_copy_rows.argtypes = [vp, vp, i64, i64, i64, i64, i32]
    lib.pmt_compose_batch.argtypes = [vp, i32, vp, i32, vp, vp, i32, i32, i32, vp, vp, vp, vp, vp, vp, vp]
    lib.pmt_compose_batch_planned.argtypes = [vp, i32, vp, i32, vp, vp, i32, vp, vp, vp, vp, vp, vp, vp]
    lib.pmt_pack_order.argtypes = [vp, vp, i32, i32, vp]
    lib.pmt_pack_order_batches.argtypes = [vp, vp, i32, i32, i32, i32, vp]
    lib.pmt_prepare_chunk.argtypes = [vp, i64, i32, i32, i32, i32, C.c_uint64, i32, i32, i32, vp, vp, vp, vp, i64, vp, vp]
    lib.pmt_layered_backward_scratch_floats.argtypes = [P(PmtModel), i64, i32]
    lib.pmt_layered_backward_scratch_floats.restype = C.c_size_t
    lib.pmt_backward_layered.argtypes = [P(PmtModel), vp, vp, vp, vp, P(PmtBatch), P(PmtOutputs), P(PmtOutputGrads), vp, vp, vp,
                                         vp, vp, vp, i32, vp]
    lib.pmt_downsample_counts.argtypes = [P(PmtDownsample), vp, vp, vp, vp, vp]
    lib.pmt_downsample_index.argtypes = [P(PmtDownsample), vp, vp, vp, vp, vp, vp]
    lib.pmt_downsample_fit.argtypes = [vp, i32, vp, vp, vp, vp, i32, C.c_double, C.c_double, C.c_double, C.c_double, C.c_double, vp, vp]
    lib.pmt_spectra_fit.argtypes = [vp, vp, vp, i32, vp, vp, i32, i32, C.c_double, C.c_double, C.c_double, C.c_double, vp]
    lib.pmt_posterior_forward.argtypes = [P(PmtPosteriorRows), i64, i64, P(PmtPosteriorParams), vp, vp, vp, vp, vp]
    lib.pmt_posterior_step.argtypes = [P(PmtPosteriorRows), i64, i64, P(PmtPosteriorParams), vp, i32, vp]
    lib.pmt_posterior_update.argtypes = [vp, i32, i64, vp, vp, vp, i64, C.c_double, C.c_double, C.c_double, C.c_double, vp, vp, vp]
    lib.pmt_balance_step.argtypes = [P(PmtBalanceArgs), vp]
    lib.pmt_record_evaluation.argtypes = [P(PmtEvalArgs), vp, vp]
    lib.pmt_posterior_rows.argtypes = [vp, i64, i32, i32, vp, vp, i32, vp, i32, vp, i64, vp]
    lib.pmt_losses_forward.argtypes = [P(PmtLossArgs), P(PmtLossOutputs), vp]
    lib.pmt_losses_backward.argtypes = [P(PmtLossArgs), P(PmtLossOutputs), P(PmtLossInputGrads), vp]
    lib.pmt_phi_forward.argtypes = [P(PmtPhiProgram), vp, vp, vp]
    lib.pmt_phi_backward.argtypes = [P(PmtPhiProgram), vp, vp, vp, vp, vp]
    for name in EXPORTS:
        fn = getattr(lib, name)
        if name not in ("pmt_abi_version", "pmt_stash_bytes", "pmt_rows_stash_bytes", "pmt_layered_scratch_floats",
                        "pmt_layered_backward_scratch_floats", "pmt_cnn_stash_floats", "pmt_cnn_workspace_floats",
                        "pmt_rows_workspace_floats"):
            fn.restype = i32
    lib.pmt_struct_bytes.argtypes = [i32]
    if lib.pmt_abi_version() != ABI_VERSION:
        raise PmtError("libpermutect_amd.so ABI version mismatch; rebuild it")
    for which, st in enumerate([PmtModel, PmtBatch, PmtOutputs, PmtOutputGrads, PmtAdamW, PmtLinear, PmtOp, PmtMlp,
                                PmtBlock, PmtHead, PmtPhiProgram, PmtLossArgs, PmtDownsample, PmtRecordArgs, PmtBalanceArgs, PmtEvalArgs,
                                PmtPosteriorRows, PmtPosteriorParams]):
        if lib.pmt_struct_bytes(which) != C.sizeof(st):
            raise PmtError(f"ctypes layout of {st.__name__} ({C.sizeof(st)} B) does not match the library "
                           f"({lib.pmt_struct_bytes(which)} B)")
    lib.pmt_shape_info.argtypes = [P(i32)]
    lib.pmt_shape_id.argtypes = [P(PmtModel)]
    lib.pmt_build_id.argtypes = [C.c_char_p, i32]
    if limits_of(lib)["group_waves"] != GROUP_WAVES:
        raise PmtError(f"{path} is built for {limits_of(lib)['group_waves']} waves per workgroup, the host side plans for {GROUP_WAVES} "
                       "(PMT_GROUP_WAVES in the environment must match a development build loaded through PMT_LIB)")
    _libs[path] = lib
    if path == LIB_PATH:
        _lib = lib
    return lib


def raw_stream(device=None) -> int:
    import torch
    idx = torch.cuda.current_device() if device is None or getattr(device, "index", None) is None else device.index
    return torch._C._cuda_getCurrentRawStream(idx)


def limits_of(lib: C.CDLL) -> dict:
    v = (i32 * 4)()
    check(lib.pmt_limits(v), "pmt_limits")
    return {"max_width": int(v[0]), "max_half_ffn": int(v[1]), "slot_floats": int(v[2]), "group_waves": int(v[3])}


def build_id(lib: C.CDLL) -> str:
    buf = C.create_string_buffer(32)
    check(lib.pmt_build_id(buf, 32), "pmt_build_id")
    return buf.value.decode()


def shape_of(lib: C.CDLL):
    v = (i32 * 9)()
    check(lib.pmt_shape_info(v), "pmt_shape_info")
    return tuple(int(x) for x in v)
```

permutect_amd/engine/plan.py:

```python
from __future__ import annotations

import ctypes as C
import os
from typing import Dict, List, Optional

import torch
from torch import nn

from permutect_amd.architecture import modules as M
from permutect_amd.engine import lib as L


def _split0(h: int) -> int:
    return 16 * ((h + 15) // 16)


def _ceil16(n: int) -> int:
    return (n + 15) // 16 * 16


class ParamSpace:

    LATE_PREFIXES = ("info_embedding.", "haplotypes_cnn.")

    @classmethod
    def is_late(cls, name: str) -> bool:
        return name.startswith(cls.LATE_PREFIXES) or name.endswith(".original")

    def __init__(self, module: nn.Module, device: torch.device):
        named = list(module.named_parameters())
        named = [(n, p) for n, p in named if not self.is_late(n)] + [(n, p) for n, p in named if self.is_late(n)]
        params = [p for _, p in named]
        self.offsets: Dict[int, int] = {}
        off = 0
        self.late_start = None
        for n, p in named:
            assert p.dtype == torch.float32, "the engine computes in fp32 (reference data/datum.py:37-38)"
            if self.late_start is None and self.is_late(n):
                self.late_start = off
            self.offsets[id(p)] = off
            off += (p.numel() + 3) // 4 * 4
        self.size = max(off, 4)
        if self.late_start is None:
            self.late_start = self.size
        self.theta = torch.zeros(self.size, dtype=torch.float32, device=device)
        self.gtheta = torch.zeros(self.size, dtype=torch.float32, device=device)
        self.params = params
        with torch.no_grad():
            for p in params:
                o, n = self.offsets[id(p)], p.numel()
                self.theta[o:o + n].copy_(p.detach().reshape(-1))
                p.data = self.theta[o:o + n].view(p.shape)
        self.bind_grads()

    def bind_grads(self, quick: bool = False):
        views = getattr(self, "_grad_views", None)
        if views is None:
            views = self._grad_views = [self.gtheta[self.offsets[id(p)]:self.offsets[id(p)] + p.numel()].view(p.shape) for p in self.params]
        if quick and self.params and self.params[0].grad is views[0] and self.params[-1].grad is views[-1]:
            return
        for p, v in zip(self.params, views):
            if p.grad is not v:
                p.grad = v

    def offset_of(self, p: nn.Parameter) -> int:
        return self.offsets[id(p)]


class EnginePlan:

    def __init__(self, model, space: ParamSpace, device: torch.device):
        self.device = device
        self.space = space
        d = L.PmtModel()
        d.abi_version = L.ABI_VERSION
        self.desc = d
        self._packed_off = 0
        self._n_lin = 0
        self._phi_off = 0
        self._phi_prog = None
        self.phi_layout: List[tuple] = []
        self.bn_folds: List[tuple] = []
        self.cnn_bn_folds: List[tuple] = []

        read_mlp: M.MLP = model.read_embedding
        enc: M.GatedRefAltMLP = model.ref_alt_reads_encoder
        reducer: M.MLP = model.reducer
        fc: M.FeatureClustering = model.feature_clustering
        d.num_read_features = read_mlp.input_dimension()
        d.read_embed_dim = read_mlp.output_dimension()
        d.d_model = enc.dimension
        d.variant_embed_dim = d.d_model - d.read_embed_dim
        d.d_ffn = enc.d_ffn
        d.num_blocks = len(enc.blocks)
        d.feature_dim = reducer.output_dimension()
        d.num_clusters = fc.num_artifact_clusters
        h, e, k = d.d_ffn // 2, d.feature_dim, d.num_clusters
        if d.num_blocks > L.MAX_BLOCKS:
            raise L.PmtError(f"{d.num_blocks} gated blocks exceed the kernel limit {L.MAX_BLOCKS}")

        self._lower_mlp(d.read_mlp, read_mlp)
        for i, blk in enumerate(enc.blocks):
            b = d.blocks[i]
            s = blk.sgu
            b.norm_w_src, b.norm_b_src = space.offset_of(blk.norm.weight), space.offset_of(blk.norm.bias)
            b.sgu_norm_w_src, b.sgu_norm_b_src = space.offset_of(s.norm.weight), space.offset_of(s.norm.bias)
            b.ref_reg_src = space.offset_of(s.ref_regularizer)
            vecs = {}
            b.proj1[0], b.proj1[1] = self._add_linear_pair(
                blk.proj1_ref, blk.proj1_alt, out_split=h,
                extra_vectors=[("norm_w", _ceil16(d.d_model)), ("norm_b", _ceil16(d.d_model)), ("sgu_w", _ceil16(h)),
                               ("sgu_b", _ceil16(h)), ("rho", _ceil16(h))], out=vecs)
            b.norm_w_pvec, b.norm_b_pvec = vecs["norm_w"], vecs["norm_b"]
            b.sgu_norm_w_pvec, b.sgu_norm_b_pvec, b.ref_reg_pvec = vecs["sgu_w"], vecs["sgu_b"], vecs["rho"]
            b.proj2[0], b.proj2[1] = self._add_linear_pair(blk.proj2_ref, blk.proj2_alt)
            b.alpha_src[0], b.alpha_src[1] = space.offset_of(s.alpha_ref), space.offset_of(s.alpha_alt)
            b.beta_src[0], b.beta_src[1] = space.offset_of(s.beta_ref), space.offset_of(s.beta_alt)
            b.gamma_src = space.offset_of(s.gamma)
            b.reg_weight_phi = self._alloc_phi(f"reg_weight.{i}", 1)
        self._lower_mlp(d.reducer, reducer)
        n_readset_lin = self._n_lin
        self._lower_mlp(d.row_mlp[L.ROWS_INFO], model.info_embedding, max_in=L.MAX_ROW_INPUT)
        self._lower_mlp(d.row_mlp[L.ROWS_ALT_COUNT], model.alt_count_predictor.wrapped_module)
        if model.num_sources > 1:
            self._lower_mlp(d.row_mlp[L.ROWS_SOURCE], model.source_predictor.wrapped_module)

        tr = model.pre_clustering_transform
        d.translation_src = space.offset_of(tr.translation_e)
        q_phi = self._alloc_phi("rotation", e * e)
        vecs = {}
        d.rotation_lin = self._add_raw_linear(e, e, w_src=-(q_phi + 2), b_src=-1, has_bias=False,
                                              extra_vectors=[("translation", _ceil16(e))], out=vecs)
        d.translation_pvec = vecs["translation"]

        hd = d.head
        hd.stdev_e_phi = self._alloc_phi("stdev_e", e)
        hd.dirs_ke_phi = self._alloc_phi("dirs_ke", k * e)
        hd.art_stdev_k_phi = self._alloc_phi("art_stdev_k", k)
        hd.log_w_k_phi = self._alloc_phi("log_w_k", k)
        hd.sigma_k_phi = self._alloc_phi("sigma_k", k)
        hd.lambda_k_phi = self._alloc_phi("lambda_k", k)
        hd.mu_k_src = space.offset_of(fc.artifact_emg.mu_k)

        self._lower_cnn(d.cnn, model.haplotypes_cnn, model.haplotypes_length() // 2)
        d.n_linear = self._n_lin
        for i in range(self._n_lin):
            lin = d.lin[i]
            out_v = _split0(lin.out_split) + lin.out_split if lin.out_split else lin.out_dim
            nmt, nkt = (out_v + 15) // 16, (lin.in_dim + 15) // 16
            lin.wb_frag = self._alloc_packed(nmt * ((nkt + 1) // 2) * 3 * 256 + 256)
            lin.wtb_frag = self._alloc_packed(nkt * ((nmt + 1) // 2) * 3 * 256 + 256)
            lin.wh_frag = self._alloc_packed(nmt * ((nkt + 1) // 2) * 2 * 256 + 256)
        d.emit_base = self._packed_off
        for i in range(d.n_linear):
            lin = d.lin[i]
            lin.emit_tab = -1
            if i >= n_readset_lin and i != d.rotation_lin:
                continue
            out_v = _split0(lin.out_split) + lin.out_split if lin.out_split > 0 else lin.out_dim
            nmt, nkt = (out_v + 15) // 16, (lin.in_dim + 15) // 16
            lin.emit_tab = self._alloc_packed(nmt * nkt * 256 + nmt * 16)
        d.emit_len = self._packed_off - d.emit_base
        d.theta_size, d.phi_size, d.packed_size = space.size, max(self._phi_off, 4), self._packed_off + 512
        d.force_shape = {"tile": 1, "any": 2, "bf16": 3, "bf16x3": 5}.get(os.environ.get("PMT_SHAPE", ""), 0)
        d.force_cnn = {"general": 1, "wave": 2, "batched": 3}.get(os.environ.get("PMT_CNN", ""), 0)
        d.cnn_debug = int(os.environ.get("PMT_CNN_DBG", "0"))
        d.dropout_p = max((float(getattr(m, "dropout_p", 0.0)) for m in model.modules() if isinstance(m, M.MLP)), default=0.0)

        from permutect_amd.engine.instances import library_for
        lib = self.lib = library_for(d)
        L.check(lib.pmt_model_check(C.byref(d)), "pmt_model_check")
        self.packed = torch.zeros(d.packed_size, dtype=torch.float32, device=device)
        rows = torch.cuda.get_device_properties(device).multi_processor_count if torch.device(device).type == "cuda" else 0
        rows = int(os.environ.get("PMT_GRAD_PARTIALS", rows))
        self.partial_rows = rows if d.emit_len > 0 else 0
        self.grad_partials = torch.zeros(max(self.partial_rows * d.emit_len, 4), dtype=torch.float32, device=device)
        self.gphi_size = d.phi_size
        raw = bytes(d)
        self.desc_dev = torch.frombuffer(bytearray(raw), dtype=torch.uint8).to(device)
        self.debug_flags = torch.zeros(64 + 8 * 512, dtype=torch.int32, device=device)
        self.stash_slots = (d.read_mlp.n_ops - 1) + (d.num_blocks + 1) + (d.reducer.n_ops - 1) + d.num_blocks

    def _alloc_packed(self, n: int) -> int:
        off = self._packed_off
        self._packed_off += (n + 3) // 4 * 4
        return off

    def _alloc_phi(self, name: str, n: int) -> int:
        off = self._phi_off
        self.phi_layout.append((name, off, n))
        self._phi_off += n
        return off

    def _close_region(self, start: int) -> int:
        n = (self._packed_off - start + 255) // 256 * 256
        self._packed_off = start + n
        return n

    def _add_raw_linear(self, in_dim: int, out_dim: int, w_src: int, b_src: int, has_bias: bool, out_split: int = 0,
                        alloc: bool = True, extra_vectors=(), out=None, max_in: int = L.MAX_WIDTH_WIDE) -> int:
        if self._n_lin >= L.MAX_LINEAR:
            raise L.PmtError("too many linear layers for the kernel descriptor")
        if in_dim > max_in or out_dim > L.MAX_WIDTH_WIDE:
            raise L.PmtError(f"layer width {in_dim}->{out_dim} exceeds the register-resident limit {L.MAX_WIDTH_WIDE}")
        lin = self.desc.lin[self._n_lin]
        out_v = _split0(out_split) + out_split if out_split else out_dim
        nmt, nkt = (out_v + 15) // 16, (in_dim + 15) // 16
        lin.in_dim, lin.out_dim, lin.out_split = in_dim, out_dim, out_split
        if alloc:
            self._packed_off = (self._packed_off + 255) // 256 * 256
            lin.w_frag = self._alloc_packed(nmt * nkt * 256)
            lin.b_pvec = self._alloc_packed(nmt * 16) if has_bias else -1
            for name, n in extra_vectors:
                out[name] = self._alloc_packed(n)
            self._close_region(lin.w_frag)
            lin.wt_frag = self._alloc_packed(nmt * nkt * 256)
        lin.w_src, lin.b_src = w_src, b_src
        self._n_lin += 1
        return self._n_lin - 1

    def _add_linear_pair(self, ref: nn.Linear, alt: nn.Linear, out_split: int = 0, extra_vectors=(), out=None):
        ids = []
        for layer in (ref, alt):
            ids.append(self._add_raw_linear(layer.in_features, layer.out_features, self.space.offset_of(layer.weight),
                                            self.space.offset_of(layer.bias), True, out_split, alloc=False))
        lr, la = self.desc.lin[ids[0]], self.desc.lin[ids[1]]
        out_v = _split0(out_split) + out_split if out_split else lr.out_dim
        nfl = ((out_v + 15) // 16) * ((lr.in_dim + 15) // 16) * 256
        nb = ((out_v + 15) // 16) * 16
        self._packed_off = (self._packed_off + 255) // 256 * 256
        lr.w_frag = self._alloc_packed(nfl); la.w_frag = self._alloc_packed(nfl)
        lr.b_pvec = self._alloc_packed(nb); la.b_pvec = self._alloc_packed(nb)
        for name, n in extra_vectors:
            out[name] = self._alloc_packed(n)
        self._close_region(lr.w_frag)
        lr.wt_frag = self._alloc_packed(nfl); la.wt_frag = self._alloc_packed(nfl)
        return ids[0], ids[1]

    def _add_linear(self, layer: nn.Linear, out_split: int = 0, max_in: int = L.MAX_WIDTH_WIDE, bn: Optional[nn.BatchNorm1d] = None) -> int:
        if bn is not None:
            n = self._n_lin
            w_phi = self._alloc_phi(f"bnfold.w.{n}", layer.out_features * layer.in_features)
            b_phi = self._alloc_phi(f"bnfold.b.{n}", layer.out_features)
            self.bn_folds.append((bn, layer))
            return self._add_raw_linear(layer.in_features, layer.out_features, -(w_phi + 2), -(b_phi + 2), True, out_split, max_in=max_in)
        b_src = self.space.offset_of(layer.bias) if layer.bias is not None else -1
        return self._add_raw_linear(layer.in_features, layer.out_features, self.space.offset_of(layer.weight), b_src,
                                    layer.bias is not None, out_split, max_in=max_in)

    def _lower_mlp(self, dst: L.PmtMlp, mlp: M.MLP, max_in: int = L.MAX_WIDTH_WIDE):
        dst.dropout = int(any(isinstance(c, nn.Dropout) for c in mlp._model.modules()))
        def strip(seq):
            kept, bn_of, pending = [], {}, None
            for m in seq:
                if isinstance(m, nn.Dropout):
                    continue
                if isinstance(m, nn.BatchNorm1d):
                    pending = m
                    continue
                if pending is not None:
                    if not isinstance(m, nn.Linear):
                        raise L.PmtError("a BatchNorm1d that is not directly in front of a Linear")
                    bn_of[m] = pending
                    pending = None
                kept.append(m)
            return kept, bn_of
        children, bn_of = strip(mlp._model.children())
        ops = []
        i = 0
        while i < len(children):
            c = children[i]
            if isinstance(c, nn.Linear):
                selu_after = i + 1 < len(children) and isinstance(children[i + 1], nn.SELU)
                ops.append(("lin", c, selu_after))
                i += 2 if selu_after else 1
            elif isinstance(c, M.DenseSkipBlock):
                inner, inner_bn = strip(c.mlp._model.children())
                bn_of.update(inner_bn)
                lins = [m for m in inner if isinstance(m, nn.Linear)]
                assert len(inner) == 2 * len(lins) and all(isinstance(m, nn.SELU) for m in inner[0::2])
                ops.append(("skip", c, lins))
                i += 1
            else:
                raise L.PmtError(f"unsupported layer in MLP: {type(c).__name__}")
        if len(ops) > L.MAX_OPS:
            raise L.PmtError(f"MLP with {len(ops)} top-level ops exceeds the kernel limit {L.MAX_OPS}")
        dst.n_ops, dst.in_dim, dst.out_dim = len(ops), mlp.input_dimension(), mlp.output_dimension()
        for j, op in enumerate(ops):
            o = dst.ops[j]
            if op[0] == "lin":
                o.kind, o.n_layers, o.selu_after, o.alpha_src = L.OP_LINEAR, 1, int(op[2]), -1
                o.lin[0] = self._add_linear(op[1], max_in=max_in if j == 0 else L.MAX_WIDTH_WIDE, bn=bn_of.get(op[1]))
            else:
                blk, lins = op[1], op[2]
                if len(lins) > L.MAX_SKIP_LAYERS:
                    raise L.PmtError(f"skip blocks deeper than {L.MAX_SKIP_LAYERS} layers are not supported by the gfx950 kernels")
                o.kind, o.n_layers, o.selu_after = L.OP_SKIP, len(lins), 0
                o.alpha_src = self.space.offset_of(blk.alpha)
                for t, lin in enumerate(lins):
                    o.lin[t] = self._add_linear(lin, bn=bn_of.get(lin))

    def _lower_cnn(self, dst: L.PmtCnn, cnn: M.DNASequenceConvolution, seq_len: int):
        layers = self._strip_cnn_batchnorm(list(cnn._model.children()))
        if len(layers) > L.MAX_CNN_LAYERS:
            raise L.PmtError(f"haplotype CNN with {len(layers)} layers exceeds the kernel limit {L.MAX_CNN_LAYERS}")
        ch, length = M.INITIAL_NUM_CHANNELS, seq_len
        off = ch * length
        in_off, max_act = 0, ch * length
        for i, layer in enumerate(layers):
            c = dst.layers[i]
            c.in_ch, c.in_len, c.in_off = ch, length, in_off
            c.kernel, c.stride, c.padding, c.dilation = 1, 1, 0, 1
            c.w_src = c.b_src = c.lin = -1
            if isinstance(layer, nn.Conv1d):
                if layer.groups != 1 or layer.padding_mode != "zeros" or isinstance(layer.padding, str):
                    raise L.PmtError("unsupported Conv1d options in the haplotype CNN")
                c.kind = L.CNN_CONV
                c.kernel, c.stride, c.padding, c.dilation = layer.kernel_size[0], layer.stride[0], layer.padding[0], layer.dilation[0]
                c.w_src, c.b_src = self.space.offset_of(layer.weight), self.space.offset_of(layer.bias)
                c.lin = self._add_raw_linear(ch * c.kernel, layer.out_channels, c.w_src, c.b_src, True, max_in=L.MAX_CNN_TAPS)
                ch, length = layer.out_channels, M._conv_len(length, kernel_size=c.kernel, stride=c.stride, padding=c.padding, dilation=c.dilation)
            elif isinstance(layer, nn.MaxPool1d):
                if layer.padding != 0 or layer.dilation != 1 or layer.ceil_mode:
                    raise L.PmtError("unsupported MaxPool1d options in the haplotype CNN")
                c.kind = L.CNN_POOL
                c.kernel = layer.kernel_size
                c.stride = layer.stride if layer.stride is not None else layer.kernel_size
                length = M._pool_len(length, kernel_size=c.kernel, stride=c.stride)
            elif isinstance(layer, (nn.LeakyReLU, nn.SELU)):
                c.kind = L.CNN_LEAKY_RELU if isinstance(layer, nn.LeakyReLU) else L.CNN_SELU
                c.out_ch, c.out_len, c.out_off = ch, length, in_off
                continue
            elif isinstance(layer, nn.Flatten):
                c.kind = L.CNN_FLATTEN
                ch, length = ch * length, 1
                c.out_ch, c.out_len, c.out_off = ch, length, in_off
                continue
            elif isinstance(layer, nn.Linear):
                c.kind = L.CNN_LINEAR
                c.w_src, c.b_src = self.space.offset_of(layer.weight), self.space.offset_of(layer.bias)
                ch, length = layer.out_features, 1
            else:
                raise L.PmtError(f"unsupported layer in the haplotype CNN: {type(layer).__name__}")
            c.out_ch, c.out_len, c.out_off = ch, length, off
            in_off = off
            off += ch * length
            max_act = max(max_act, ch * length)
        dst.n_layers, dst.seq_len, dst.out_dim = len(layers), seq_len, ch * length
        dst.max_act, dst.sum_act = max_act, off

    def _strip_cnn_batchnorm(self, layers):
        kept = []
        for i, layer in enumerate(layers):
            if not isinstance(layer, nn.BatchNorm1d):
                kept.append(layer)
                continue
            prev = layers[i - 1] if i > 0 else None
            if isinstance(prev, (nn.Conv1d, nn.Linear)):
                self.cnn_bn_folds.append((layer, prev, "out", 1))
                continue
            j = i + 1
            while j < len(layers) and isinstance(layers[j], nn.Flatten):
                j += 1
            nxt = layers[j] if j < len(layers) else None
            if isinstance(nxt, nn.Conv1d) and nxt.padding[0] == 0 and nxt.in_channels == layer.num_features:
                self.cnn_bn_folds.append((layer, nxt, "in", 1))
            elif isinstance(nxt, nn.Linear) and nxt.in_features % layer.num_features == 0:
                self.cnn_bn_folds.append((layer, nxt, "in", nxt.in_features // layer.num_features))
            else:
                raise L.PmtError("a batch_norm token of the haplotype CNN that is neither directly behind a convolution / linear nor in "
                                 "front of an un-padded convolution / a linear cannot be folded (permutect_amd runs it in eval mode only)")
        return kept

    def folded_cnn_theta(self, theta: torch.Tensor) -> torch.Tensor:
        out = theta.detach().clone()
        space = self.space
        with torch.no_grad():
            for bn, layer, side, per in self.cnn_bn_folds:
                s = bn.weight / torch.sqrt(bn.running_var + bn.eps)
                t = bn.bias - bn.running_mean * s
                wo, bo = space.offset_of(layer.weight), space.offset_of(layer.bias)
                w = out[wo:wo + layer.weight.numel()].view_as(layer.weight)
                b = out[bo:bo + layer.bias.numel()]
                if side == "out":
                    b.mul_(s).add_(t)
                    w.mul_(s.view(-1, *([1] * (w.dim() - 1))))
                elif w.dim() == 3:
                    b.add_((w * t.view(1, -1, 1)).sum(dim=(1, 2)))
                    w.mul_(s.view(1, -1, 1))
                else:
                    se, te = s.repeat_interleave(per), t.repeat_interleave(per)
                    b.add_(w @ te)
                    w.mul_(se.view(1, -1))
        return out

    def phi_program(self, model):
        tr, fc, space = model.pre_clustering_transform, model.feature_clustering, self.space
        e = self.desc.feature_dim
        if e > L.MAX_ORTHO_DIM or self.bn_folds:
            return None
        if self._phi_prog is None:
            offs = {name: off for name, off, _ in self.phi_layout}
            prog = L.PmtPhiProgram()
            segs = []

            def original(mod, name):
                return space.offset_of(getattr(mod.parametrizations, name).original)

            def bounded(mod, name):
                p = getattr(mod.parametrizations, name)[0]
                return float(p.min_val), float(p.size)

            for i, blk in enumerate(model.ref_alt_reads_encoder.blocks):
                segs.append((L.PHI_EXP, original(blk.sgu, "reg_weight"), offs[f"reg_weight.{i}"], 1, 1, 0.0, 0.0))
            segs.append((L.PHI_ORTHOGONAL, original(tr.rotation_ee, "weight"), offs["rotation"], e, e, 0.0, 0.0))
            k = self.desc.num_clusters
            segs.append((L.PHI_BOUNDED, original(fc, "nonartifact_stdev_e"), offs["stdev_e"], 1, e) + bounded(fc, "nonartifact_stdev_e"))
            segs.append((L.PHI_UNIT_ROWS, original(fc, "artifact_directions_ke"), offs["dirs_ke"], k, e, 0.0, 0.0))
            segs.append((L.PHI_BOUNDED, original(fc, "artifact_stdev_k"), offs["art_stdev_k"], 1, k) + bounded(fc, "artifact_stdev_k"))
            segs.append((L.PHI_LOG_SOFTMAX, original(fc, "log_cluster_weights_k"), offs["log_w_k"], 1, k, 0.0, 0.0))
            segs.append((L.PHI_BOUNDED, original(fc.artifact_emg, "sigma_k"), offs["sigma_k"], 1, k) + bounded(fc.artifact_emg, "sigma_k"))
            segs.append((L.PHI_BOUNDED, original(fc.artifact_emg, "lambda_k"), offs["lambda_k"], 1, k) + bounded(fc.artifact_emg, "lambda_k"))
            assert len(segs) <= L.MAX_PHI_SEGS
            prog.n_segs = len(segs)
            for sg, (kind, toff, poff, rows, cols, p0, p1) in zip(prog.seg, segs):
                sg.kind, sg.theta_off, sg.phi_off, sg.rows, sg.cols, sg.p0, sg.p1 = kind, toff, poff, rows, cols, p0, p1
            self._phi_prog = prog
            self._phi_rot_index = len(model.ref_alt_reads_encoder.blocks)
        base = getattr(tr.rotation_ee.parametrizations.weight[0], "base", None)
        sg = self._phi_prog.seg[self._phi_rot_index]
        if base is None:
            sg.base, sg.base_rs, sg.base_cs = None, 0, 0
        else:
            sg.base, sg.base_rs, sg.base_cs = base.data_ptr(), base.stride(0), base.stride(1)
        return self._phi_prog

    def materialize_phi(self, model) -> torch.Tensor:
        fc = model.feature_clustering
        vals = {f"reg_weight.{i}": blk.sgu.reg_weight for i, blk in enumerate(model.ref_alt_reads_encoder.blocks)}
        vals.update({"rotation": model.pre_clustering_transform.rotation_ee.weight, "stdev_e": fc.nonartifact_stdev_e,
                     "dirs_ke": fc.artifact_directions_ke, "art_stdev_k": fc.artifact_stdev_k, "log_w_k": fc.log_cluster_weights_k,
                     "sigma_k": fc.artifact_emg.sigma_k, "lambda_k": fc.artifact_emg.lambda_k})
        names = [n for n, _, _ in self.phi_layout if n.startswith("bnfold.w.")]
        for name, (bn, lin) in zip(names, self.bn_folds):
            s = bn.weight / torch.sqrt(bn.running_var + bn.eps)
            t = bn.bias - bn.running_mean * s
            vals[name] = lin.weight * s[None, :]
            vals["bnfold.b." + name[len("bnfold.w."):]] = lin.bias + lin.weight @ t
        parts, at = [], 0
        for name, off, n in self.phi_layout:
            assert off == at and vals[name].numel() == n, (name, off, at)
            parts.append(vals[name].reshape(-1))
            at += n
        phi = torch.cat(parts)
        if phi.numel() < self.desc.phi_size:
            phi = torch.cat([phi, phi.new_zeros(self.desc.phi_size - phi.numel())])
        return phi
```

permutect_amd/engine/runtime.py:

```python
from __future__ import annotations

import ctypes as C
import os
from typing import Optional, Tuple

import torch
from torch import Tensor

from permutect_amd.engine import lib as L
from permutect_amd.engine.plan import EnginePlan, ParamSpace


def _ptr(t: Optional[Tensor]) -> Optional[int]:
    return None if t is None else t.data_ptr()


def _stream() -> int:
    return L.raw_stream()


class ReadSetEngine:
    def __init__(self, model, device: torch.device):
        if device.type != "cuda":
            raise L.PmtError("permutect_amd computes on an MI355X (ROCm device 'cuda') only; there is no CPU fallback. "
                             "Model construction, state_dict and save/load work on any device.")
        self.device = device
        self.space = ParamSpace(model, device)
        self.plan = EnginePlan(model, self.space, device)
        self.lib = self.plan.lib
        self.shape_id = int(self.lib.pmt_shape_id(C.byref(self.plan.desc)))
        self._trigger = torch.zeros(1, dtype=torch.float32, device=device, requires_grad=True)
        self._no_trigger = torch.zeros(1, dtype=torch.float32, device=device)
        self._cnn_ws = None
        self._rows_ws = None
        self.join_layered = os.environ.get("PMT_LAYERED_JOIN", "1") != "0"
        self.dropout_seed = 0
        self.join_fault = torch.zeros(1, dtype=torch.int32, device=device)
        self._param_epoch = 0
        self.packed_for = None
        self.timers = None
        self.timer_stride, self._timer_calls = 1, {}
        self.grad_hook = None

    def _event_start(self, name: str):
        if self.timers is None:
            return None
        n = self._timer_calls.get(name, 0)
        self._timer_calls[name] = n + 1
        if n % max(1, int(self.timer_stride)) != 0:
            return None
        ev = torch.cuda.Event(enable_timing=True)
        ev.record()
        return ev

    def _event_stop(self, name: str, start):
        if start is not None:
            end = torch.cuda.Event(enable_timing=True)
            end.record()
            self.timers[name].append((start, end))

    def check_join_fault(self):
        word = int(self.join_fault.item())
        if word != 0:
            self.join_fault.zero_()
            what = []
            if word & 1:
                what.append("a joined layered launch timed out waiting for the other workgroups of a split read set "
                            "(PMT_LAYERED_JOIN=0 runs the layered launches instead)")
            if word & 2:
                what.append("an activation left the range of the forward's f16 operand pieces (|x| > 65504 where the residual stream enters the "
                            "reducer or its output the rotation): those operands saturate (PMT_SHAPE=bf16x3 runs the bf16-piece forward, which has no such limit)")
            if word & 4:
                what.append("the device-side group planner of a downsampled batch ran out of its group capacity (pmt_plan_groups_device)")
            raise L.PmtError("; ".join(what) + ": the logits / gradients computed since the last check are wrong")

    def params_changed(self):
        self._param_epoch += 1

    def params_key(self):
        try:
            stats = sum(bn.running_mean._version + bn.running_var._version
                        for bn in [f[0] for f in self.plan.bn_folds] + [f[0] for f in self.plan.cnn_bn_folds])
            return (self._param_epoch, self.space.theta._version, sum(p._version for p in self.space.params), stats)
        except RuntimeError:
            return None

    def pack(self, phi: Tensor):
        d = self.plan
        L.check(self.lib.pmt_pack_params(C.byref(d.desc), d.desc_dev.data_ptr(), self.space.theta.data_ptr(),
                                         phi.data_ptr(), d.packed.data_ptr(), _stream()), "pmt_pack_params")

    def cnn_params(self) -> Tuple[Tensor, Tensor]:
        if not self.plan.cnn_bn_folds:
            return self.space.theta, self.plan.packed
        key = self.params_key()
        if key is None or getattr(self, "_cnn_fold_key", None) != key:
            theta_f = self.plan.folded_cnn_theta(self.space.theta)
            packed_f = torch.zeros_like(self.plan.packed)
            phi0 = torch.zeros(max(self.plan.desc.phi_size, 4), dtype=torch.float32, device=self.device)
            L.check(self.lib.pmt_pack_params(C.byref(self.plan.desc), self.plan.desc_dev.data_ptr(), theta_f.data_ptr(), phi0.data_ptr(),
                                             packed_f.data_ptr(), _stream()), "pmt_pack_params")
            self._cnn_fold, self._cnn_fold_key = (theta_f, packed_f), key
        return self._cnn_fold

    def cnn_workspace(self) -> Optional[Tensor]:
        if self._cnn_ws is None:
            n = self.lib.pmt_cnn_workspace_floats(C.byref(self.plan.desc)) if os.environ.get("PMT_CNN_WORKSPACE", "1") != "0" else 0
            self._cnn_ws = torch.empty(n, dtype=torch.float32, device=self.device) if n > 0 else False
        return self._cnn_ws if self._cnn_ws is not False else None

    def rows_workspace(self) -> Optional[Tensor]:
        if self._rows_ws is None:
            n = 0
            if os.environ.get("PMT_ROWS_WORKSPACE", "1") != "0":
                n = max(self.lib.pmt_rows_workspace_floats(C.byref(self.plan.desc), w) if self.plan.desc.row_mlp[w].n_ops > 0 else 0
                        for w in range(3))
            self._rows_ws = torch.zeros(n, dtype=torch.float32, device=self.device) if n > 0 else False
        return self._rows_ws if self._rows_ws is not False else None

    def offsets(self, batch) -> Tuple[Tensor, Tensor]:
        if getattr(batch, "_offsets", None) is None:
            ref_c, alt_c, elem, stride = batch.device_counts()
            b = batch.size()
            ref_off = torch.empty(b + 1, dtype=torch.int32, device=self.device)
            alt_off = torch.empty(b + 1, dtype=torch.int32, device=self.device)
            L.check(self.lib.pmt_scan_counts(ref_c.data_ptr(), alt_c.data_ptr(), elem, stride, b, ref_off.data_ptr(),
                                             alt_off.data_ptr(), _stream()), "pmt_scan_counts")
            batch._offsets = (ref_off, alt_off)
        return batch._offsets

    @property
    def trigger(self) -> Tensor:
        return self._trigger if torch.is_grad_enabled() else self._no_trigger

    def draw_dropout_seed(self, training: bool) -> int:
        self.dropout_seed = int(torch.randint(1, 2 ** 62, (1,)).item()) if (training and self.plan.desc.dropout_p > 0) else 0
        return self.dropout_seed

    def batch_view(self, batch, variant_embed: Tensor, allow_split: bool = True, dropout_seed: int = 0):
        plan = batch.plan(allow_split=allow_split, fault=self.join_fault)
        gs, gt, span = plan.on(self.device)
        ref_off, alt_off = self.offsets(batch)
        reads, fmt, row_bytes, index = batch.read_rows()
        if reads.device != self.device:
            raise L.PmtError("batch tensors must be on the model's device (call batch.copy_to(device, dtype))")
        bv = L.PmtBatch()
        bv.num_variants, bv.num_groups = batch.size(), plan.num_groups
        bv.read_format, bv.read_row_bytes = fmt, row_bytes
        bv.reads, bv.read_index = reads.data_ptr(), _ptr(index)
        bv.ref_offsets, bv.alt_offsets = ref_off.data_ptr(), alt_off.data_ptr()
        bv.variant_embed = variant_embed.data_ptr()
        bv.group_start, bv.group_tile_base = gs.data_ptr(), gt.data_ptr()
        bv.total_tiles = plan.total_tiles
        bv.debug_flags = self.plan.debug_flags.data_ptr()
        bv.group_span = _ptr(span)
        bv.num_groups_dev = _ptr(getattr(plan, "num_groups_dev", None))
        sets = plan.set_groups_on(self.device) if (getattr(plan, "set_groups", None) is not None and self.join_layered) else None
        bv.set_groups = _ptr(sets)
        bv.dropout_seed = dropout_seed
        bv.join_fault = self.join_fault.data_ptr()
        keep = (gs, gt, span, ref_off, alt_off, reads, index, variant_embed, sets)
        return bv, keep, plan

    def forward(self, batch, phi: Tensor, variant_embed: Tensor, train: bool, dropout_seed: int = 0):
        d = self.plan.desc
        b, k, e = batch.size(), d.num_clusters, d.feature_dim
        variant_embed = variant_embed.contiguous().float()
        assert variant_embed.shape == (b, d.variant_embed_dim), (variant_embed.shape, d.variant_embed_dim)
        phi = phi.contiguous()
        bv, keep, plan = self.batch_view(batch, variant_embed, dropout_seed=dropout_seed)
        dev = self.device
        logits_b = torch.empty(b, dtype=torch.float32, device=dev)
        logits_bk = torch.empty(b, k + 2, dtype=torch.float32, device=dev)
        feats = torch.empty(b, e, dtype=torch.float32, device=dev)
        ref_feats = torch.empty(b, e, dtype=torch.float32, device=dev)
        out = L.PmtOutputs(logits_b.data_ptr(), logits_bk.data_ptr(), feats.data_ptr(), ref_feats.data_ptr())
        stash = None
        if train:
            nbytes = self.lib.pmt_stash_bytes(C.byref(d), plan.total_tiles, b)
            stash = torch.empty(nbytes // 4, dtype=torch.float32, device=dev)
        ev = self._event_start("pmt_forward")
        if plan.layered:
            scratch = torch.empty(self.lib.pmt_layered_scratch_floats(C.byref(d), plan.total_tiles, b), dtype=torch.float32, device=dev)
            L.check(self.lib.pmt_forward_layered(C.byref(d), self.plan.desc_dev.data_ptr(), self.space.theta.data_ptr(),
                                                 phi.data_ptr(), self.plan.packed.data_ptr(), C.byref(bv), C.byref(out),
                                                 _ptr(stash), scratch.data_ptr(), _stream()), "pmt_forward_layered")
        else:
            L.check(self.lib.pmt_forward(C.byref(d), self.plan.desc_dev.data_ptr(), self.space.theta.data_ptr(),
                                         phi.data_ptr(), self.plan.packed.data_ptr(), C.byref(bv), C.byref(out),
                                         _ptr(stash), _stream()), "pmt_forward")
        self._event_stop("pmt_forward", ev)
        return (logits_b, logits_bk, feats, ref_feats), stash, variant_embed, phi

    def backward(self, batch, phi: Tensor, variant_embed: Tensor, stash: Tensor, outs, grads, dropout_seed: int = 0):
        d = self.plan.desc
        bv, keep, plan = self.batch_view(batch, variant_embed, dropout_seed=dropout_seed)
        g = [None if t is None else t.contiguous().float() for t in grads]
        dout = L.PmtOutputGrads(_ptr(g[0]), _ptr(g[1]), _ptr(g[2]), _ptr(g[3]))
        out = L.PmtOutputs(*[t.data_ptr() for t in outs])
        gphi = torch.zeros(d.phi_size, dtype=torch.float32, device=self.device)
        gvar = torch.zeros_like(variant_embed) if plan.layered else torch.empty_like(variant_embed)
        ev = self._event_start("pmt_backward")
        if plan.layered:
            n = self.lib.pmt_layered_backward_scratch_floats(C.byref(d), plan.total_tiles, batch.size())
            scratch = torch.empty(n, dtype=torch.float32, device=self.device)
            L.check(self.lib.pmt_backward_layered(C.byref(d), self.plan.desc_dev.data_ptr(), self.space.theta.data_ptr(),
                                                  phi.data_ptr(), self.plan.packed.data_ptr(), C.byref(bv), C.byref(out),
                                                  C.byref(dout), stash.data_ptr(), scratch.data_ptr(),
                                                  self.space.gtheta.data_ptr(), gphi.data_ptr(), gvar.data_ptr(),
                                                  self.plan.grad_partials.data_ptr(), self.plan.partial_rows, _stream()),
                    "pmt_backward_layered")
        else:
            L.check(self.lib.pmt_backward(C.byref(d), self.plan.desc_dev.data_ptr(), self.space.theta.data_ptr(),
                                          phi.data_ptr(), self.plan.packed.data_ptr(), C.byref(bv), C.byref(out),
                                          C.byref(dout), stash.data_ptr(), self.space.gtheta.data_ptr(), gphi.data_ptr(),
                                          gvar.data_ptr(), self.plan.grad_partials.data_ptr(), self.plan.partial_rows, _stream()),
                    "pmt_backward")
        self._event_stop("pmt_backward", ev)
        if self.grad_hook is not None:
            self.grad_hook.early(self.space.gtheta, self.space.late_start)
        return gphi, gvar


class LossesFunction(torch.autograd.Function):

    @staticmethod
    def _args(engine, logits_b, logits_bk, alt_raw, source_logits, labels, alt_counts, sources, weights, source_weights):
        from permutect_amd import constants
        a = L.PmtLossArgs()
        a.num_variants, a.num_clusters = logits_b.shape[0], logits_bk.shape[1] - 2
        a.num_sources = 1 if source_logits is None else source_logits.shape[1]
        a.max_outlier_logit, a.max_alt_count = constants.MAX_OUTLIER_LOGIT, float(constants.MAX_ALT_COUNT)
        a.logits_b, a.logits_bk, a.alt_count_raw = logits_b.data_ptr(), logits_bk.data_ptr(), alt_raw.data_ptr()
        a.source_logits = _ptr(source_logits)
        a.labels, a.label_stride = labels.data_ptr(), labels.stride(0)
        a.alt_counts, a.alt_count_stride = alt_counts.data_ptr(), alt_counts.stride(0)
        a.sources, a.source_stride = _ptr(sources), (0 if sources is None else sources.stride(0))
        a.weights, a.source_weights = weights.data_ptr(), source_weights.data_ptr()
        return a

    @staticmethod
    def forward(ctx, engine, logits_b, logits_bk, alt_raw, source_logits, labels, alt_counts, sources, weights, source_weights):
        alt_shape = alt_raw.shape
        logits_b, logits_bk, alt_raw = logits_b.contiguous(), logits_bk.contiguous(), alt_raw.contiguous().view(-1)
        source_logits = None if source_logits is None else source_logits.contiguous()
        weights, source_weights = weights.contiguous().float(), source_weights.contiguous().float()
        assert labels.dtype == torch.int64 and alt_counts.dtype == torch.int64 and (sources is None or sources.dtype == torch.int64)
        b = logits_b.shape[0]
        outs = [torch.empty(b, dtype=torch.float32, device=logits_b.device) for _ in range(5)]
        a = LossesFunction._args(engine, logits_b, logits_bk, alt_raw, source_logits, labels, alt_counts, sources, weights, source_weights)
        o = L.PmtLossOutputs(*[t.data_ptr() for t in outs])
        L.check(engine.lib.pmt_losses_forward(C.byref(a), C.byref(o), _stream()), "pmt_losses_forward")
        ctx.engine = engine
        ctx.alt_shape = alt_shape
        ctx.set_materialize_grads(False)
        ctx.save_for_backward(logits_b, logits_bk, alt_raw, labels, alt_counts, weights, source_weights,
                              *(() if source_logits is None else (source_logits, sources)))
        return tuple(outs)

    @staticmethod
    def backward(ctx, *grads):
        saved = ctx.saved_tensors
        logits_b, logits_bk, alt_raw, labels, alt_counts, weights, source_weights = saved[:7]
        source_logits, sources = (saved[7], saved[8]) if len(saved) > 7 else (None, None)
        grads = [None if g is None else g.contiguous().float() for g in grads]
        a = LossesFunction._args(ctx.engine, logits_b, logits_bk, alt_raw, source_logits, labels, alt_counts, sources, weights, source_weights)
        g = L.PmtLossOutputs(*[_ptr(t) for t in grads])
        d_b, d_bk, d_alt = torch.empty_like(logits_b), torch.empty_like(logits_bk), torch.empty_like(alt_raw)
        d_src = None if source_logits is None else torch.empty_like(source_logits)
        d = L.PmtLossInputGrads(d_b.data_ptr(), d_bk.data_ptr(), d_alt.data_ptr(), _ptr(d_src))
        L.check(ctx.engine.lib.pmt_losses_backward(C.byref(a), C.byref(g), C.byref(d), _stream()), "pmt_losses_backward")
        return None, d_b, d_bk, d_alt.view(ctx.alt_shape), d_src, None, None, None, None, None


class PhiFunction(torch.autograd.Function):

    @staticmethod
    def forward(ctx, engine: "ReadSetEngine", prog, trigger: Tensor):
        phi = torch.zeros(engine.plan.desc.phi_size, dtype=torch.float32, device=engine.device)
        L.check(engine.lib.pmt_phi_forward(C.byref(prog), engine.space.theta.data_ptr(), phi.data_ptr(), _stream()), "pmt_phi_forward")
        ctx.engine, ctx.prog = engine, prog
        ctx.save_for_backward(phi)
        return phi

    @staticmethod
    def backward(ctx, gphi: Tensor):
        (phi,) = ctx.saved_tensors
        eng = ctx.engine
        gphi = gphi.contiguous()
        L.check(eng.lib.pmt_phi_backward(C.byref(ctx.prog), eng.space.theta.data_ptr(), phi.data_ptr(), gphi.data_ptr(),
                                         eng.space.gtheta.data_ptr(), _stream()), "pmt_phi_backward")
        return None, None, None


class ReadSetFunction(torch.autograd.Function):

    @staticmethod
    def forward(ctx, engine: ReadSetEngine, batch, phi: Tensor, variant_embed: Tensor):
        train = bool(ctx.needs_input_grad[2] or ctx.needs_input_grad[3])
        ctx.dropout_seed = engine.dropout_seed
        outs, stash, ve, ph = engine.forward(batch, phi.detach(), variant_embed.detach(), train, ctx.dropout_seed)
        ctx.engine, ctx.batch, ctx.train = engine, batch, train
        ctx.set_materialize_grads(False)
        if train:
            ctx.save_for_backward(ph, ve, stash, *outs)
        return outs

    @staticmethod
    def backward(ctx, d_logits_b, d_logits_bk, d_feats, d_ref_feats):
        if not ctx.train:
            return None, None, None, None
        phi, ve, stash, *outs = ctx.saved_tensors
        ctx.engine.space.bind_grads(quick=True)
        gphi, gvar = ctx.engine.backward(ctx.batch, phi, ve, stash, outs, (d_logits_b, d_logits_bk, d_feats, d_ref_feats),
                                         ctx.dropout_seed)
        return None, None, gphi, gvar


class HaplotypeCnnFunction(torch.autograd.Function):

    @staticmethod
    def forward(ctx, engine: ReadSetEngine, haplotypes: Tensor, trigger: Tensor):
        d = engine.plan.desc
        hap = haplotypes if haplotypes.dtype == torch.int64 else haplotypes.long()
        assert hap.stride(-1) == 1 and hap.shape[1] == 2 * d.cnn.seq_len
        n = hap.shape[0]
        out = torch.empty(n, d.cnn.out_dim, dtype=torch.float32, device=engine.device)
        train = bool(ctx.needs_input_grad[2])
        per = engine.lib.pmt_cnn_stash_floats(C.byref(d)) if train and os.environ.get("PMT_CNN_STASH", "1") != "0" else 0
        stash = torch.empty(n * per, dtype=torch.float32, device=engine.device) if per > 0 and n > 0 else None
        if train and engine.plan.cnn_bn_folds:
            raise NotImplementedError("a haplotype CNN with batch_norm tokens runs under no_grad / inference_mode only (its BatchNorms are folded "
                                      "into the neighbouring layers' weights); a backward through it is not built")
        cnn_theta, cnn_packed = engine.cnn_params()
        L.check(engine.lib.pmt_cnn_forward(C.byref(d), engine.plan.desc_dev.data_ptr(), cnn_theta.data_ptr(),
                                           cnn_packed.data_ptr(), hap.data_ptr(), hap.stride(0), n, out.data_ptr(), out.stride(0),
                                           _ptr(stash), _stream()),
                "pmt_cnn_forward")
        ctx.engine, ctx.train, ctx.stash = engine, train, stash
        ctx.hap = hap
        return out

    @staticmethod
    def backward(ctx, d_out):
        if not ctx.train:
            return None, None, None
        eng, d, hap = ctx.engine, ctx.engine.plan.desc, ctx.hap
        eng.space.bind_grads(quick=True)
        if d_out.dtype != torch.float32 or d_out.stride(-1) != 1:
            d_out = d_out.float().contiguous()
        ws = eng.cnn_workspace()
        L.check(eng.lib.pmt_cnn_backward(C.byref(d), eng.plan.desc_dev.data_ptr(), eng.space.theta.data_ptr(),
                                         eng.plan.packed.data_ptr(), hap.data_ptr(), hap.stride(0), hap.shape[0], d_out.data_ptr(), d_out.stride(0),
                                         _ptr(ctx.stash), eng.space.gtheta.data_ptr(), _ptr(ws), 0 if ws is None else ws.numel(), _stream()),
                "pmt_cnn_backward")
        ctx.stash = None
        return None, None, None


class VariantEmbedFunction(torch.autograd.Function):

    @staticmethod
    def forward(ctx, engine: ReadSetEngine, info: Tensor, haplotypes: Tensor, trigger: Tensor):
        lib, d = engine.lib, engine.plan.desc
        mlp = d.row_mlp[L.ROWS_INFO]
        n = info.shape[0]
        x = info.detach()
        if x.dtype != torch.float32 or x.stride(-1) != 1:
            x = x.float().contiguous()
        hap = haplotypes if haplotypes.dtype == torch.int64 else haplotypes.long()
        assert x.shape[1] == mlp.in_dim and hap.stride(-1) == 1 and hap.shape[1] == 2 * d.cnn.seq_len
        e_info, e_hap = mlp.out_dim, d.cnn.out_dim
        ve = torch.empty(n, e_info + e_hap, dtype=torch.float32, device=engine.device)
        train = bool(ctx.needs_input_grad[3])
        rows_stash = cnn_stash = None
        if train:
            rows_stash = torch.empty(lib.pmt_rows_stash_bytes(C.byref(d), L.ROWS_INFO, n) // 4, dtype=torch.float32, device=engine.device)
            per = lib.pmt_cnn_stash_floats(C.byref(d)) if os.environ.get("PMT_CNN_STASH", "1") != "0" else 0
            cnn_stash = torch.empty(n * per, dtype=torch.float32, device=engine.device) if per > 0 and n > 0 else None
        L.check(lib.pmt_rows_forward(C.byref(d), engine.plan.desc_dev.data_ptr(), L.ROWS_INFO, engine.space.theta.data_ptr(),
                                     engine.plan.packed.data_ptr(), x.data_ptr(), x.stride(0), n, ve.data_ptr(), ve.stride(0),
                                     _ptr(rows_stash), engine.dropout_seed, _stream()), "pmt_rows_forward")
        if train and engine.plan.cnn_bn_folds:
            raise NotImplementedError("a haplotype CNN with batch_norm tokens runs under no_grad / inference_mode only (its BatchNorms are folded "
                                      "into the neighbouring layers' weights); a backward through it is not built")
        cnn_theta, cnn_packed = engine.cnn_params()
        L.check(lib.pmt_cnn_forward(C.byref(d), engine.plan.desc_dev.data_ptr(), cnn_theta.data_ptr(),
                                    cnn_packed.data_ptr(), hap.data_ptr(), hap.stride(0), n, ve.data_ptr() + 4 * e_info, ve.stride(0),
                                    _ptr(cnn_stash), _stream()), "pmt_cnn_forward")
        ctx.engine, ctx.train, ctx.dropout_seed, ctx.e_info = engine, train, engine.dropout_seed, e_info
        ctx.hap, ctx.cnn_stash = hap, cnn_stash
        if train:
            ctx.save_for_backward(x, rows_stash)
        return ve

    @staticmethod
    def backward(ctx, d_ve):
        if not ctx.train:
            return None, None, None, None
        x, rows_stash = ctx.saved_tensors
        eng, d, hap = ctx.engine, ctx.engine.plan.desc, ctx.hap
        eng.space.bind_grads(quick=True)
        if d_ve.dtype != torch.float32 or d_ve.stride(-1) != 1:
            d_ve = d_ve.float().contiguous()
        n = x.shape[0]
        ws = eng.rows_workspace()
        L.check(eng.lib.pmt_rows_backward(C.byref(d), eng.plan.desc_dev.data_ptr(), L.ROWS_INFO, eng.space.theta.data_ptr(),
                                          eng.plan.packed.data_ptr(), x.data_ptr(), x.stride(0), n, d_ve.data_ptr(), d_ve.stride(0),
                                          rows_stash.data_ptr(), eng.space.gtheta.data_ptr(), None, 0, 1.0, _ptr(ws),
                                          0 if ws is None else ws.numel(), ctx.dropout_seed, _stream()), "pmt_rows_backward")
        cws = eng.cnn_workspace()
        L.check(eng.lib.pmt_cnn_backward(C.byref(d), eng.plan.desc_dev.data_ptr(), eng.space.theta.data_ptr(),
                                         eng.plan.packed.data_ptr(), hap.data_ptr(), hap.stride(0), n, d_ve.data_ptr() + 4 * ctx.e_info,
                                         d_ve.stride(0), _ptr(ctx.cnn_stash), eng.space.gtheta.data_ptr(), _ptr(cws),
                                         0 if cws is None else cws.numel(), _stream()), "pmt_cnn_backward")
        ctx.cnn_stash = None
        return None, None, None, None


class RowsMlpFunction(torch.autograd.Function):

    @staticmethod
    def forward(ctx, engine: ReadSetEngine, which: int, x: Tensor, trigger: Tensor, reverse_alpha: Optional[float]):
        lib, d = engine.lib, engine.plan.desc
        mlp = d.row_mlp[which]
        n = x.shape[0]
        x = x.detach()
        if x.dtype != torch.float32 or x.stride(-1) != 1:
            x = x.float().contiguous()
        assert x.shape[1] == mlp.in_dim
        out = torch.empty(n, mlp.out_dim, dtype=torch.float32, device=engine.device)
        train = bool(ctx.needs_input_grad[2] or ctx.needs_input_grad[3])
        stash = None
        if train:
            stash = torch.empty(lib.pmt_rows_stash_bytes(C.byref(d), which, n) // 4, dtype=torch.float32, device=engine.device)
        L.check(lib.pmt_rows_forward(C.byref(d), engine.plan.desc_dev.data_ptr(), which, engine.space.theta.data_ptr(),
                                     engine.plan.packed.data_ptr(), x.data_ptr(), x.stride(0), n, out.data_ptr(),
                                     out.stride(0), _ptr(stash), engine.dropout_seed, _stream()), "pmt_rows_forward")
        ctx.dropout_seed = engine.dropout_seed
        ctx.engine, ctx.which, ctx.train, ctx.alpha = engine, which, train, reverse_alpha
        ctx.x_needs_grad = bool(ctx.needs_input_grad[2])
        if train:
            ctx.save_for_backward(x, stash)
        return out

    @staticmethod
    def backward(ctx, d_out):
        if not ctx.train:
            return None, None, None, None, None
        x, stash = ctx.saved_tensors
        eng, d = ctx.engine, ctx.engine.plan.desc
        eng.space.bind_grads(quick=True)
        if d_out.dtype != torch.float32 or d_out.stride(-1) != 1:
            d_out = d_out.float().contiguous()
        n = x.shape[0]
        d_in = torch.empty_like(x) if ctx.x_needs_grad else None
        scale = 1.0 if ctx.alpha is None else -float(ctx.alpha)
        ws = eng.rows_workspace()
        L.check(eng.lib.pmt_rows_backward(C.byref(d), eng.plan.desc_dev.data_ptr(), ctx.which, eng.space.theta.data_ptr(),
                                          eng.plan.packed.data_ptr(), x.data_ptr(), x.stride(0), n, d_out.data_ptr(),
                                          d_out.stride(0), stash.data_ptr(), eng.space.gtheta.data_ptr(), _ptr(d_in),
                                          d_in.stride(0) if d_in is not None else 0, scale, _ptr(ws), 0 if ws is None else ws.numel(),
                                          ctx.dropout_seed, _stream()), "pmt_rows_backward")
        return None, None, d_in, None, None
```

Before: 19.44 million.

## Fuse loss total reduction into losses kernel and drop default weight tensors

```diff
diff --git a/include/permutect_amd.h b/include/permutect_amd.h
--- a/include/permutect_amd.h
+++ b/include/permutect_amd.h
@@ -227,7 +227,8 @@
     const float* base;
 } PmtPhiSeg;
 typedef struct PmtPhiProgram {
-    int32_t n_segs, reserved;
+    int32_t n_segs;
+    int32_t phi_size;
     PmtPhiSeg seg[PMT_MAX_PHI_SEGS];
 } PmtPhiProgram;
 
@@ -326,6 +327,11 @@
 } PmtLossInputGrads;
 int pmt_losses_forward(const PmtLossArgs* args, const PmtLossOutputs* out, void* stream);
 int pmt_losses_backward(const PmtLossArgs* args, const PmtLossOutputs* grad_out, const PmtLossInputGrads* grad_in, void* stream);
+size_t pmt_losses_scratch_bytes(int32_t num_variants);
+int pmt_losses_forward_total(const PmtLossArgs* args, const PmtLossOutputs* out, float* total, void* scratch, size_t scratch_bytes,
+                             void* stream);
+int pmt_losses_backward_total(const PmtLossArgs* args, const PmtLossOutputs* grad_out, const float* grad_total,
+                              const PmtLossInputGrads* grad_in, void* stream);
 
 typedef struct PmtRecordArgs {
     int32_t num_variants, num_bins;
diff --git a/permutect_amd/architecture/artifact_model.py b/permutect_amd/architecture/artifact_model.py
--- a/permutect_amd/architecture/artifact_model.py
+++ b/permutect_amd/architecture/artifact_model.py
@@ -30,8 +30,28 @@
         self.ref_features_be = ref_features_be
         self.logits_b = logits_b
         self.logits_bk = logits_bk
-        self.weights = weights
-        self.source_weights = source_weights
+        self._weights = weights
+        self._source_weights = source_weights
+
+    @property
+    def weights(self) -> Tensor:
+        if self._weights is None:
+            self._weights = torch.ones_like(self.logits_b)
+        return self._weights
+
+    @weights.setter
+    def weights(self, value: Tensor):
+        self._weights = value
+
+    @property
+    def source_weights(self) -> Tensor:
+        if self._source_weights is None:
+            self._source_weights = torch.ones_like(self.logits_b)
+        return self._source_weights
+
+    @source_weights.setter
+    def source_weights(self, value: Tensor):
+        self._source_weights = value
 
     @property
     def artifact_probs_b(self) -> Tensor:
@@ -47,13 +67,13 @@
 class BatchLosses:
 
     def __init__(self, supervised_losses_b, unsupervised_losses_b, alt_count_losses_b, source_prediction_losses_b,
-                 total_losses_b):
+                 total_losses_b, total_loss=None):
         self.supervised_losses_b = supervised_losses_b
         self.unsupervised_losses_b = unsupervised_losses_b
         self.alt_count_losses_b = alt_count_losses_b
         self.source_prediction_losses_b = source_prediction_losses_b
         self.total_losses_b = total_losses_b
-        self.total_loss = torch.sum(total_losses_b)
+        self.total_loss = torch.sum(total_losses_b) if total_loss is None else total_loss
 
 
 class SetMeansView:
@@ -181,7 +201,7 @@
     def compute_batch_output(self, batch: Batch, balancer=None) -> BatchOutput:
         (logits_b, logits_bk, feats, ref_feats), _ = self._encode(batch)
         if balancer is None:
-            weights_b = source_weights = torch.ones_like(logits_b)
+            weights_b = source_weights = torch.ones_like(logits_b) if self.engine().step_tail_legacy else None
         elif logits_b.is_cuda and hasattr(balancer, "weights_from_logits"):
             weights_b, source_weights = balancer.weights_from_logits(batch, logits_b)
         else:
@@ -218,10 +238,10 @@
             source_logits = RowsMlpFunction.apply(eng, L.ROWS_SOURCE, output.features_be, eng.trigger,
                                                   float(self.source_predictor.gradient_reversal.alpha))
             sources = batch.get(Data.SOURCE).long()
-        sup, unsup, alt, src, total = LossesFunction.apply(
+        sup, unsup, alt, src, total, total_loss = LossesFunction.apply(
             eng, output.logits_b, output.logits_bk, alt_raw, source_logits, batch.get(Data.LABEL).long(),
-            batch.get(Data.ALT_COUNT).long(), sources, output.weights, output.source_weights)
-        return BatchLosses(sup, unsup, alt, src, total)
+            batch.get(Data.ALT_COUNT).long(), sources, output._weights, output._source_weights)
+        return BatchLosses(sup, unsup, alt, src, total, total_loss)
 
     def compute_batch_losses_torch(self, output: BatchOutput, batch: Batch) -> BatchLosses:
         labels_b = batch.get_training_labels()
diff --git a/permutect_amd/csrc/pmt_losses.hip b/permutect_amd/csrc/pmt_losses.hip
--- a/permutect_amd/csrc/pmt_losses.hip
+++ b/permutect_amd/csrc/pmt_losses.hip
@@ -1,5 +1,6 @@
 #include <hip/hip_runtime.h>
 #include <math.h>
+#include <stdint.h>
 
 #include "permutect_amd.h"
 
@@ -22,9 +23,7 @@
     return r;
 }
 
-__global__ __launch_bounds__(LOSS_THREADS) void pmt_losses_forward_kernel(PmtLossArgs a, PmtLossOutputs out) {
-    const int b = blockIdx.x * LOSS_THREADS + threadIdx.x;
-    if (b >= a.num_variants) return;
+__device__ __forceinline__ float losses_of_variant(const PmtLossArgs& a, const PmtLossOutputs& out, int b) {
     const int K = a.num_clusters, S = a.num_sources;
     const long long label = a.labels[(size_t)b * a.label_stride];
     const float is_labeled = label != 2 ? 1.f : 0.f;
@@ -53,18 +52,68 @@
     out.unsupervised_b[b] = unsup;
     out.alt_count_b[b] = altl;
     out.source_b[b] = src;
-    out.total_b[b] = a.weights[b] * (sup + unsup + altl) + a.source_weights[b] * src;
-}
-
-__global__ __launch_bounds__(LOSS_THREADS) void pmt_losses_backward_kernel(PmtLossArgs a, PmtLossOutputs g, PmtLossInputGrads d) {
+    const float w = a.weights ? a.weights[b] : 1.f, sw = a.source_weights ? a.source_weights[b] : 1.f;
+    const float total = w * (sup + unsup + altl) + sw * src;
+    out.total_b[b] = total;
+    return total;
+}
+
+__global__ __launch_bounds__(LOSS_THREADS) void pmt_losses_forward_kernel(PmtLossArgs a, PmtLossOutputs out, float* total,
+                                                                          double* partials, unsigned* counter) {
+    const int b = blockIdx.x * LOSS_THREADS + threadIdx.x;
+    float mine = 0.f;
+    if (b < a.num_variants) mine = losses_of_variant(a, out, b);
+    if (total == nullptr) return;
+    __shared__ double sh[LOSS_THREADS + 1];
+    double v = (double)mine;
+    for (int d = 32; d > 0; d >>= 1) v += __shfl_down(v, d, 64);
+    if ((threadIdx.x & 63) == 0) sh[threadIdx.x >> 6] = v;
+    __syncthreads();
+    if (threadIdx.x == 0) {
+        double sum = sh[0];
+        for (int w = 1; w < LOSS_THREADS / 64; ++w) sum += sh[w];
+        __hip_atomic_store(&partials[blockIdx.x], sum, __ATOMIC_RELAXED, __HIP_MEMORY_SCOPE_AGENT);
+        asm volatile("s_waitcnt vmcnt(0)" ::: "memory");
+        __builtin_amdgcn_fence(__ATOMIC_RELEASE, "agent");
+        asm volatile("s_waitcnt vmcnt(0)" ::: "memory");
+        const unsigned arrival = __hip_atomic_fetch_add(counter, 1u, __ATOMIC_RELAXED, __HIP_MEMORY_SCOPE_AGENT);
+        const bool last = arrival == gridDim.x - 1;
+        if (last) {
+            __builtin_amdgcn_fence(__ATOMIC_ACQUIRE, "agent");
+            asm volatile("s_waitcnt vmcnt(0)" ::: "memory");
+        }
+        sh[LOSS_THREADS] = last ? 1.0 : 0.0;
+    }
+    __syncthreads();
+    if (sh[LOSS_THREADS] == 0.0) return;
+    double sum = 0.0;
+    for (unsigned base = 0; base < gridDim.x; base += LOSS_THREADS) {
+        const unsigned i = base + threadIdx.x;
+        __syncthreads();
+        sh[threadIdx.x] = i < gridDim.x ? __hip_atomic_load(&partials[i], __ATOMIC_RELAXED, __HIP_MEMORY_SCOPE_AGENT) : 0.0;
+        __syncthreads();
+        if (threadIdx.x == 0) {
+            const unsigned n = min((unsigned)LOSS_THREADS, gridDim.x - base);
+            for (unsigned k = 0; k < n; ++k) sum += sh[k];
+        }
+    }
+    if (threadIdx.x == 0) {
+        *total = (float)sum;
+        __hip_atomic_store(counter, 0u, __ATOMIC_RELAXED, __HIP_MEMORY_SCOPE_AGENT);
+    }
+}
+
+__global__ __launch_bounds__(LOSS_THREADS) void pmt_losses_backward_kernel(PmtLossArgs a, PmtLossOutputs g, PmtLossInputGrads d,
+                                                                           const float* g_total) {
     const int b = blockIdx.x * LOSS_THREADS + threadIdx.x;
     if (b >= a.num_variants) return;
     const int K = a.num_clusters, S = a.num_sources;
-    const float gt = g.total_b ? g.total_b[b] : 0.f;
-    const float g_sup = (g.supervised_b ? g.supervised_b[b] : 0.f) + gt * a.weights[b];
-    const float g_unsup = (g.unsupervised_b ? g.unsupervised_b[b] : 0.f) + gt * a.weights[b];
-    const float g_alt = (g.alt_count_b ? g.alt_count_b[b] : 0.f) + gt * a.weights[b];
-    const float g_src = (g.source_b ? g.source_b[b] : 0.f) + gt * a.source_weights[b];
+    const float gt = (g.total_b ? g.total_b[b] : 0.f) + (g_total ? *g_total : 0.f);
+    const float w = a.weights ? a.weights[b] : 1.f, sw = a.source_weights ? a.source_weights[b] : 1.f;
+    const float g_sup = (g.supervised_b ? g.supervised_b[b] : 0.f) + gt * w;
+    const float g_unsup = (g.unsupervised_b ? g.unsupervised_b[b] : 0.f) + gt * w;
+    const float g_alt = (g.alt_count_b ? g.alt_count_b[b] : 0.f) + gt * w;
+    const float g_src = (g.source_b ? g.source_b[b] : 0.f) + gt * sw;
     const long long label = a.labels[(size_t)b * a.label_stride];
     const float is_labeled = label != 2 ? 1.f : 0.f;
     const float target = label == 0 ? 1.f : (label == 2 ? 0.5f : 0.f);
@@ -102,31 +151,63 @@
 static int loss_args_check(const PmtLossArgs* a) {
     if (!a || a->num_variants < 0 || a->num_clusters < 0 || a->num_clusters > PMT_MAX_CLUSTERS || a->num_sources < 1) return PMT_E_INVALID;
     if (a->num_variants == 0) return PMT_OK;
-    if (!a->logits_b || !a->logits_bk || !a->alt_count_raw || !a->labels || !a->alt_counts || !a->weights || !a->source_weights)
-        return PMT_E_INVALID;
+    if (!a->logits_b || !a->logits_bk || !a->alt_count_raw || !a->labels || !a->alt_counts) return PMT_E_INVALID;
     if (a->num_sources > 1 && a->source_logits && !a->sources) return PMT_E_INVALID;
     return PMT_OK;
 }
 
-extern "C" int pmt_losses_forward(const PmtLossArgs* args, const PmtLossOutputs* out, void* stream) {
+#define LOSS_SCRATCH_HEAD 16
+static int losses_blocks(int num_variants) { return (num_variants + LOSS_THREADS - 1) / LOSS_THREADS; }
+
+extern "C" size_t pmt_losses_scratch_bytes(int32_t num_variants) {
+    return LOSS_SCRATCH_HEAD + sizeof(double) * (size_t)(num_variants > 0 ? losses_blocks(num_variants) : 1);
+}
+
+static int losses_forward(const PmtLossArgs* args, const PmtLossOutputs* out, float* total, void* scratch, void* stream) {
     const int rc = loss_args_check(args);
     if (rc) return rc;
     if (!out || !out->supervised_b || !out->unsupervised_b || !out->alt_count_b || !out->source_b || !out->total_b) return PMT_E_INVALID;
-    if (args->num_variants == 0) return PMT_OK;
-    hipLaunchKernelGGL(pmt_losses_forward_kernel, dim3((args->num_variants + LOSS_THREADS - 1) / LOSS_THREADS), dim3(LOSS_THREADS), 0,
-                       reinterpret_cast<hipStream_t>(stream), *args, *out);
-    return hipGetLastError() == hipSuccess ? PMT_OK : PMT_E_LAUNCH;
-}
-
-extern "C" int pmt_losses_backward(const PmtLossArgs* args, const PmtLossOutputs* grad_out, const PmtLossInputGrads* grad_in,
-                                   void* stream) {
+    hipStream_t s = reinterpret_cast<hipStream_t>(stream);
+    if (args->num_variants == 0) {
+        if (total && hipMemsetAsync(total, 0, sizeof(float), s) != hipSuccess) return PMT_E_LAUNCH;
+        return PMT_OK;
+    }
+    char* sc = reinterpret_cast<char*>(scratch);
+    hipLaunchKernelGGL(pmt_losses_forward_kernel, dim3(losses_blocks(args->num_variants)), dim3(LOSS_THREADS), 0, s, *args, *out, total,
+                       reinterpret_cast<double*>(sc ? sc + LOSS_SCRATCH_HEAD : nullptr), reinterpret_cast<unsigned*>(sc));
+    return hipGetLastError() == hipSuccess ? PMT_OK : PMT_E_LAUNCH;
+}
+
+extern "C" int pmt_losses_forward(const PmtLossArgs* args, const PmtLossOutputs* out, void* stream) {
+    return losses_forward(args, out, nullptr, nullptr, stream);
+}
+
+extern "C" int pmt_losses_forward_total(const PmtLossArgs* args, const PmtLossOutputs* out, float* total, void* scratch, size_t scratch_bytes,
+                                        void* stream) {
+    if (!args || !total || !scratch || (reinterpret_cast<uintptr_t>(scratch) & 15) != 0) return PMT_E_INVALID;
+    if (scratch_bytes < pmt_losses_scratch_bytes(args->num_variants)) return PMT_E_WORKSPACE;
+    return losses_forward(args, out, total, scratch, stream);
+}
+
+static int losses_backward(const PmtLossArgs* args, const PmtLossOutputs* grad_out, const float* grad_total, const PmtLossInputGrads* grad_in,
+                           void* stream) {
     const int rc = loss_args_check(args);
     if (rc) return rc;
     if (!grad_out || !grad_in || !grad_in->d_logits_b || !grad_in->d_logits_bk || !grad_in->d_alt_count_raw) return PMT_E_INVALID;
     if (args->num_variants == 0) return PMT_OK;
-    hipLaunchKernelGGL(pmt_losses_backward_kernel, dim3((args->num_variants + LOSS_THREADS - 1) / LOSS_THREADS), dim3(LOSS_THREADS), 0,
-                       reinterpret_cast<hipStream_t>(stream), *args, *grad_out, *grad_in);
-    return hipGetLastError() == hipSuccess ? PMT_OK : PMT_E_LAUNCH;
+    hipLaunchKernelGGL(pmt_losses_backward_kernel, dim3(losses_blocks(args->num_variants)), dim3(LOSS_THREADS), 0,
+                       reinterpret_cast<hipStream_t>(stream), *args, *grad_out, *grad_in, grad_total);
+    return hipGetLastError() == hipSuccess ? PMT_OK : PMT_E_LAUNCH;
+}
+
+extern "C" int pmt_losses_backward(const PmtLossArgs* args, const PmtLossOutputs* grad_out, const PmtLossInputGrads* grad_in,
+                                   void* stream) {
+    return losses_backward(args, grad_out, nullptr, grad_in, stream);
+}
+
+extern "C" int pmt_losses_backward_total(const PmtLossArgs* args, const PmtLossOutputs* grad_out, const float* grad_total,
+                                         const PmtLossInputGrads* grad_in, void* stream) {
+    return losses_backward(args, grad_out, grad_total, grad_in, stream);
 }
 
 #define REC_THREADS 256
diff --git a/permutect_amd/csrc/pmt_phi.hip b/permutect_amd/csrc/pmt_phi.hip
--- a/permutect_amd/csrc/pmt_phi.hip
+++ b/permutect_amd/csrc/pmt_phi.hip
@@ -81,11 +81,85 @@
     }
 }
 
+__device__ __forceinline__ double dot_rc(const double* __restrict__ A, const double* __restrict__ B, int i, int j, int N) {
+    double a0 = 0.0, a1 = 0.0, a2 = 0.0, a3 = 0.0;
+    const double* ar = A + i * N;
+    const double* bc = B + j;
+    int k = 0;
+    for (; k + 3 < N; k += 4) {
+        a0 += ar[k] * bc[k * N];
+        a1 += ar[k + 1] * bc[(k + 1) * N];
+        a2 += ar[k + 2] * bc[(k + 2) * N];
+        a3 += ar[k + 3] * bc[(k + 3) * N];
+    }
+    for (; k < N; ++k) a0 += ar[k] * bc[k * N];
+    return (a0 + a1) + (a2 + a3);
+}
+
+__device__ const double* expm_pair(double* w, int n, double* red) {
+    const int nn = n * n;
+    double *B = w, *H = w + nn, *E = w + 2 * nn, *Lm = w + 3 * nn;
+    double *Pc = w + 4 * nn, *Qc = w + 5 * nn, *Pn = w + 6 * nn, *Qn = w + 7 * nn;
+    double colsum = 0.0;
+    if (threadIdx.x < n)
+        for (int i = 0; i < n; ++i) colsum += fabs(B[i * n + threadIdx.x]);
+    const double norm1 = block_max(colsum, red);
+    int s = 0;
+    if (norm1 > 0.5) s = (int)ceil(log2(norm1 / 0.5));
+    const double scale = ldexp(1.0, -s);
+    for (int idx = threadIdx.x; idx < nn; idx += PHI_THREADS) {
+        const double b = B[idx] * scale, h = H[idx] * scale;
+        const int i = idx / n, j = idx - i * n;
+        B[idx] = b;
+        H[idx] = h;
+        Pc[idx] = b;
+        Qc[idx] = h;
+        E[idx] = b + (i == j ? 1.0 : 0.0);
+        Lm[idx] = h;
+    }
+    __syncthreads();
+    for (int k = 2; k <= 12; ++k) {
+        const double inv_k = 1.0 / (double)k;
+        for (int idx = threadIdx.x; idx < 2 * nn; idx += PHI_THREADS) {
+            const bool deriv = idx >= nn;
+            const int e = deriv ? idx - nn : idx;
+            const int i = e / n, j = e - i * n;
+            if (!deriv) {
+                const double v = dot_rc(Pc, B, i, j, n) * inv_k;
+                Pn[e] = v;
+                E[e] += v;
+            } else {
+                const double v = (dot_rc(Pc, H, i, j, n) + dot_rc(Qc, B, i, j, n)) * inv_k;
+                Qn[e] = v;
+                Lm[e] += v;
+            }
+        }
+        __syncthreads();
+        double* t = Pc; Pc = Pn; Pn = t;
+        t = Qc; Qc = Qn; Qn = t;
+    }
+    double *En = Pc, *Ln = Qc;
+    for (int q = 0; q < s; ++q) {
+        for (int idx = threadIdx.x; idx < 2 * nn; idx += PHI_THREADS) {
+            const bool deriv = idx >= nn;
+            const int e = deriv ? idx - nn : idx;
+            const int i = e / n, j = e - i * n;
+            if (!deriv) En[e] = dot_rc(E, E, i, j, n);
+            else Ln[e] = dot_rc(E, Lm, i, j, n) + dot_rc(Lm, E, i, j, n);
+        }
+        __syncthreads();
+        double* t = E; E = En; En = t;
+        t = Lm; Lm = Ln; Ln = t;
+    }
+    return Lm;
+}
+
 struct PhiShared {
     double m[4][PHI_MAXN * PHI_MAXN];
     double red[PHI_THREADS];
 };
 static_assert(sizeof(PhiShared) <= 160 * 1024, "LDS budget");
+static_assert(8 * PMT_MAX_ORTHO_DIM * PMT_MAX_ORTHO_DIM <= 4 * PHI_MAXN * PHI_MAXN, "expm_pair's eight n x n matrices live in PhiShared::m");
 
 __global__ __launch_bounds__(PHI_THREADS) void pmt_phi_forward_kernel(PmtPhiProgram prog, const float* __restrict__ theta,
                                                                        float* __restrict__ phi) {
@@ -94,6 +168,11 @@
     const float* x = theta + sg.theta_off;
     float* y = phi + sg.phi_off;
     const int tid = threadIdx.x, n = sg.rows * sg.cols;
+    if (blockIdx.x == 0 && prog.phi_size > 0) {
+        int covered = 0;
+        for (int q = 0; q < prog.n_segs; ++q) covered = max(covered, prog.seg[q].phi_off + prog.seg[q].rows * prog.seg[q].cols);
+        for (int i = covered + tid; i < prog.phi_size; i += PHI_THREADS) phi[i] = 0.f;
+    }
     if (sg.kind == PMT_PHI_EXP) {
         for (int i = tid; i < n; i += PHI_THREADS) y[i] = expf(x[i]);
     } else if (sg.kind == PMT_PHI_BOUNDED) {
@@ -176,6 +255,7 @@
                 gx[r * sg.cols + i] += (float)((double)gy[r * sg.cols + i] - exp((double)y[r * sg.cols + i]) * gsum);
         }
     } else if (sg.kind == PMT_PHI_ORTHOGONAL) {
+#if PMT_PHI_ADJOINT_2N
         const int nn = sg.rows, N = 2 * nn;
         double* S = sh.m[0];
         double* G = sh.m[1];
@@ -208,6 +288,27 @@
             const int i = idx / nn, j = idx - i * nn;
             if (i > j) gx[idx] += (float)(S[i * N + nn + j] - S[j * N + nn + i]);
         }
+#else
+        const int n1 = sg.rows, nn = n1 * n1;
+        double* w = &sh.m[0][0];
+        for (int idx = tid; idx < nn; idx += PHI_THREADS) {
+            const int i = idx / n1, j = idx - i * n1;
+            w[idx] = i > j ? -(double)x[i * n1 + j] : (i < j ? (double)x[j * n1 + i] : 0.0);
+            double acc = 0.0;
+            if (sg.base != nullptr) {
+                for (int k = 0; k < n1; ++k) acc += (double)sg.base[k * sg.base_rs + i * sg.base_cs] * (double)gy[k * n1 + j];
+            } else {
+                acc = (double)gy[idx];
+            }
+            w[nn + idx] = acc;
+        }
+        __syncthreads();
+        const double* GA = expm_pair(w, n1, sh.red);
+        for (int idx = tid; idx < nn; idx += PHI_THREADS) {
+            const int i = idx / n1, j = idx - i * n1;
+            if (i > j) gx[idx] += (float)(GA[i * n1 + j] - GA[j * n1 + i]);
+        }
+#endif
     }
 }
 
diff --git a/permutect_amd/engine/lib.py b/permutect_amd/engine/lib.py
--- a/permutect_amd/engine/lib.py
+++ b/permutect_amd/engine/lib.py
@@ -115,7 +115,7 @@
 
 
 class PmtPhiProgram(C.Structure):
-    _fields_ = [("n_segs", i32), ("reserved", i32), ("seg", PmtPhiSeg * MAX_PHI_SEGS)]
+    _fields_ = [("n_segs", i32), ("phi_size", i32), ("seg", PmtPhiSeg * MAX_PHI_SEGS)]
 
 
 class PmtIntColumn(C.Structure):
@@ -197,7 +197,7 @@
 EXPORTS = ["pmt_abi_version", "pmt_build_id", "pmt_shape_info", "pmt_shape_id", "pmt_limits", "pmt_struct_bytes", "pmt_model_check", "pmt_plan_groups", "pmt_plan_groups_device", "pmt_plan_device_chunks", "pmt_stash_bytes", "pmt_pack_params",
            "pmt_scan_counts", "pmt_forward", "pmt_backward", "pmt_clip_adamw",
            "pmt_dropout_mask", "pmt_rows_stash_bytes", "pmt_rows_forward", "pmt_rows_backward", "pmt_rows_workspace_floats", "pmt_cnn_forward", "pmt_cnn_backward", "pmt_cnn_stash_floats", "pmt_cnn_workspace_floats",
-           "pmt_phi_forward", "pmt_phi_backward", "pmt_build_read_index", "pmt_losses_forward", "pmt_losses_backward",
+           "pmt_phi_forward", "pmt_phi_backward", "pmt_build_read_index", "pmt_losses_forward", "pmt_losses_backward", "pmt_losses_scratch_bytes", "pmt_losses_forward_total", "pmt_losses_backward_total",
            "pmt_downsample_counts", "pmt_downsample_index", "pmt_downsample_fit", "pmt_spectra_fit", "pmt_posterior_forward", "pmt_posterior_step", "pmt_posterior_update", "pmt_record_losses", "pmt_record_evaluation", "pmt_balance_step", "pmt_posterior_rows",
            "pmt_plan_groups_split", "pmt_layered_scratch_floats", "pmt_forward_layered",
            "pmt_layered_backward_scratch_floats", "pmt_backward_layered", "pmt_host_copy", "pmt_pack_order", "pmt_pack_order_batches", "pmt_prepare_chunk", "pmt_host_copy_rows", "pmt_compose_batch", "pmt_compose_batch_planned"]
@@ -282,13 +282,17 @@
     lib.pmt_posterior_rows.argtypes = [vp, i64, i32, i32, vp, vp, i32, vp, i32, vp, i64, vp]
     lib.pmt_losses_forward.argtypes = [P(PmtLossArgs), P(PmtLossOutputs), vp]
     lib.pmt_losses_backward.argtypes = [P(PmtLossArgs), P(PmtLossOutputs), P(PmtLossInputGrads), vp]
+    lib.pmt_losses_scratch_bytes.argtypes = [i32]
+    lib.pmt_losses_scratch_bytes.restype = C.c_size_t
+    lib.pmt_losses_forward_total.argtypes = [P(PmtLossArgs), P(PmtLossOutputs), vp, vp, C.c_size_t, vp]
+    lib.pmt_losses_backward_total.argtypes = [P(PmtLossArgs), P(PmtLossOutputs), vp, P(PmtLossInputGrads), vp]
     lib.pmt_phi_forward.argtypes = [P(PmtPhiProgram), vp, vp, vp]
     lib.pmt_phi_backward.argtypes = [P(PmtPhiProgram), vp, vp, vp, vp, vp]
     for name in EXPORTS:
         fn = getattr(lib, name)
         if name not in ("pmt_abi_version", "pmt_stash_bytes", "pmt_rows_stash_bytes", "pmt_layered_scratch_floats",
                         "pmt_layered_backward_scratch_floats", "pmt_cnn_stash_floats", "pmt_cnn_workspace_floats",
-                        "pmt_rows_workspace_floats"):
+                        "pmt_rows_workspace_floats", "pmt_losses_scratch_bytes"):
             fn.restype = i32
     lib.pmt_struct_bytes.argtypes = [i32]
     if lib.pmt_abi_version() != ABI_VERSION:
diff --git a/permutect_amd/engine/plan.py b/permutect_amd/engine/plan.py
--- a/permutect_amd/engine/plan.py
+++ b/permutect_amd/engine/plan.py
@@ -423,6 +423,7 @@
             segs.append((L.PHI_BOUNDED, original(fc.artifact_emg, "lambda_k"), offs["lambda_k"], 1, k) + bounded(fc.artifact_emg, "lambda_k"))
             assert len(segs) <= L.MAX_PHI_SEGS
             prog.n_segs = len(segs)
+            prog.phi_size = self.desc.phi_size
             for sg, (kind, toff, poff, rows, cols, p0, p1) in zip(prog.seg, segs):
                 sg.kind, sg.theta_off, sg.phi_off, sg.rows, sg.cols, sg.p0, sg.p1 = kind, toff, poff, rows, cols, p0, p1
             self._phi_prog = prog
diff --git a/permutect_amd/engine/runtime.py b/permutect_amd/engine/runtime.py
--- a/permutect_amd/engine/runtime.py
+++ b/permutect_amd/engine/runtime.py
@@ -41,6 +41,8 @@
         self.timers = None
         self.timer_stride, self._timer_calls = 1, {}
         self.grad_hook = None
+        self.step_tail_legacy = os.environ.get("PMT_STEP_TAIL", "") == "legacy"
+        self._loss_scratch = None
 
     def _event_start(self, name: str):
         if self.timers is None:
@@ -117,6 +119,12 @@
                         for w in range(3))
             self._rows_ws = torch.zeros(n, dtype=torch.float32, device=self.device) if n > 0 else False
         return self._rows_ws if self._rows_ws is not False else None
+
+    def loss_scratch(self, b: int) -> Tensor:
+        need = int(self.lib.pmt_losses_scratch_bytes(b))
+        if self._loss_scratch is None or self._loss_scratch.numel() < need:
+            self._loss_scratch = torch.zeros(max(need, 4096), dtype=torch.uint8, device=self.device)
+        return self._loss_scratch
 
     def offsets(self, batch) -> Tuple[Tensor, Tensor]:
         if getattr(batch, "_offsets", None) is None:
@@ -236,7 +244,7 @@
         a.labels, a.label_stride = labels.data_ptr(), labels.stride(0)
         a.alt_counts, a.alt_count_stride = alt_counts.data_ptr(), alt_counts.stride(0)
         a.sources, a.source_stride = _ptr(sources), (0 if sources is None else sources.stride(0))
-        a.weights, a.source_weights = weights.data_ptr(), source_weights.data_ptr()
+        a.weights, a.source_weights = _ptr(weights), _ptr(source_weights)
         return a
 
     @staticmethod
@@ -244,23 +252,34 @@
         alt_shape = alt_raw.shape
         logits_b, logits_bk, alt_raw = logits_b.contiguous(), logits_bk.contiguous(), alt_raw.contiguous().view(-1)
         source_logits = None if source_logits is None else source_logits.contiguous()
-        weights, source_weights = weights.contiguous().float(), source_weights.contiguous().float()
+        weights = None if weights is None else weights.contiguous().float()
+        source_weights = None if source_weights is None else source_weights.contiguous().float()
         assert labels.dtype == torch.int64 and alt_counts.dtype == torch.int64 and (sources is None or sources.dtype == torch.int64)
         b = logits_b.shape[0]
         outs = [torch.empty(b, dtype=torch.float32, device=logits_b.device) for _ in range(5)]
         a = LossesFunction._args(engine, logits_b, logits_bk, alt_raw, source_logits, labels, alt_counts, sources, weights, source_weights)
         o = L.PmtLossOutputs(*[t.data_ptr() for t in outs])
-        L.check(engine.lib.pmt_losses_forward(C.byref(a), C.byref(o), _stream()), "pmt_losses_forward")
+        total = None
+        if engine.step_tail_legacy:
+            L.check(engine.lib.pmt_losses_forward(C.byref(a), C.byref(o), _stream()), "pmt_losses_forward")
+        else:
+            total = torch.empty((), dtype=torch.float32, device=logits_b.device)
+            scratch = engine.loss_scratch(b)
+            L.check(engine.lib.pmt_losses_forward_total(C.byref(a), C.byref(o), total.data_ptr(), scratch.data_ptr(), scratch.numel(), _stream()),
+                    "pmt_losses_forward_total")
         ctx.engine = engine
         ctx.alt_shape = alt_shape
         ctx.set_materialize_grads(False)
         ctx.save_for_backward(logits_b, logits_bk, alt_raw, labels, alt_counts, weights, source_weights,
                               *(() if source_logits is None else (source_logits, sources)))
-        return tuple(outs)
+        return (*outs, total)
 
     @staticmethod
     def backward(ctx, *grads):
         saved = ctx.saved_tensors
+        *grads, g_total = grads
+        if g_total is not None:
+            g_total = g_total.contiguous().float()
         logits_b, logits_bk, alt_raw, labels, alt_counts, weights, source_weights = saved[:7]
         source_logits, sources = (saved[7], saved[8]) if len(saved) > 7 else (None, None)
         grads = [None if g is None else g.contiguous().float() for g in grads]
@@ -269,7 +288,7 @@
         d_b, d_bk, d_alt = torch.empty_like(logits_b), torch.empty_like(logits_bk), torch.empty_like(alt_raw)
         d_src = None if source_logits is None else torch.empty_like(source_logits)
         d = L.PmtLossInputGrads(d_b.data_ptr(), d_bk.data_ptr(), d_alt.data_ptr(), _ptr(d_src))
-        L.check(ctx.engine.lib.pmt_losses_backward(C.byref(a), C.byref(g), C.byref(d), _stream()), "pmt_losses_backward")
+        L.check(ctx.engine.lib.pmt_losses_backward_total(C.byref(a), C.byref(g), _ptr(g_total), C.byref(d), _stream()), "pmt_losses_backward_total")
         return None, d_b, d_bk, d_alt.view(ctx.alt_shape), d_src, None, None, None, None, None
 
 
@@ -277,7 +296,8 @@
 
     @staticmethod
     def forward(ctx, engine: "ReadSetEngine", prog, trigger: Tensor):
-        phi = torch.zeros(engine.plan.desc.phi_size, dtype=torch.float32, device=engine.device)
+        make = torch.zeros if (engine.step_tail_legacy or prog.phi_size != engine.plan.desc.phi_size) else torch.empty
+        phi = make(engine.plan.desc.phi_size, dtype=torch.float32, device=engine.device)
         L.check(engine.lib.pmt_phi_forward(C.byref(prog), engine.space.theta.data_ptr(), phi.data_ptr(), _stream()), "pmt_phi_forward")
         ctx.engine, ctx.prog = engine, prog
         ctx.save_for_backward(phi)
```

Result: no change. 19.63 million, median of 6 (+1.0%).
